# usamec/GAML

Measured on AMD Instinct MI355X. Metric: reads_per_sec_scored, higher is better.
Workload: dtype f64; 1 GPU; cfg3: 5 Mbp, 50x 2x150 paired, insert 300+-30; 833333 pairs in all, whole true genome as 1-2 walks, 8 rotating path sets, window cache warm; pairs_total=833333, pairs_per_gpu=833333, genome_bp=5000000, parallelism=reads sharded over 1 GPU(s)

## Files before the change

gaml_amd/api.py:

```python
from __future__ import annotations

import ctypes as C
import importlib.util
import os
import sys

import numpy as np

_HERE = os.path.dirname(os.path.abspath(__file__))
FLAVOUR = os.environ.get("GAML_HIP_FLAVOUR", "release")
LIB_PATH = os.environ.get("GAML_HIP_LIB") or os.path.join(_HERE, "libgaml_hip_dev.so" if FLAVOUR == "dev" else "libgaml_hip.so")

OK, EINVAL, ENODEVICE, EHIP, ESTATE = 0, -1, -2, -3, -4

_i32p = np.ctypeslib.ndpointer(np.int32, flags="C_CONTIGUOUS")
_i64p = np.ctypeslib.ndpointer(np.int64, flags="C_CONTIGUOUS")
_f64p = np.ctypeslib.ndpointer(np.float64, flags="C_CONTIGUOUS")
_u8p = np.ctypeslib.ndpointer(np.uint8, flags="C_CONTIGUOUS")

ALIGMENT = np.dtype([("position", np.int32), ("edit_dist", np.int32), ("read_id", np.int32), ("orientation", np.int32)])
PACBIO_ALIGMENT = np.dtype([("position", np.int32), ("position_end", np.int32), ("read_id", np.int32), ("pad_", np.int32),
                            ("logprob", np.float64)])


# ... 585 lines not shown
        o = out[:n]
        return np.stack([o["position"], o["edit_dist"], o["read_id"], o["orientation"]], axis=1)

    def align_window(self, rs, mate, walk) -> int:
        walk = np.ascontiguousarray(walk, np.int32)
        return _lib.gaml_hip_align_window(self._h, rs, mate, walk, len(walk))

    def debug_prepare(self, paths):
        flat, offs = _flat(paths)
        self._check(_lib.gaml_hip_debug_prepare(self._h, flat, offs, len(paths)))

    def debug_occurrences(self, rs, mate=0) -> np.ndarray:
        n = _lib.gaml_hip_debug_occurrences(self._h, rs, mate, np.zeros(5, np.int32), 0)
        out = np.zeros(5 * max(1, n), np.int32)
        _lib.gaml_hip_debug_occurrences(self._h, rs, mate, out, n)
        return out.reshape(-1, 5)[:n]

    def debug_table_occurrences(self, rs, mate=0):
        info = np.zeros(3, np.int64)
        n = _lib.gaml_hip_debug_table_occurrences(self._h, rs, mate, np.zeros(5, np.int32), 0, info)
        out = np.zeros(5 * max(1, n), np.int32)
        _lib.gaml_hip_debug_table_occurrences(self._h, rs, mate, out, n, info)
        return out.reshape(-1, 5)[:n], {"incremental": bool(info[0]), "incremental_calls": int(info[1]), "full_calls": int(info[2])}

    def debug_window_walk(self, rs, mate, wid) -> list:
        buf = np.zeros(64, np.int32)
        n = _lib.gaml_hip_debug_window_walk(self._h, rs, mate, wid, buf, 64)
        if n > 64:
            buf = np.zeros(n, np.int32)
            _lib.gaml_hip_debug_window_walk(self._h, rs, mate, wid, buf, n)
        return [int(x) for x in buf[:n]]

    def table_stats(self, rs):
        out = np.zeros(10, np.int64)
        self._check(_lib.gaml_hip_table_stats(self._h, rs, out))
        return {"full_rebuilds": int(out[0]), "delta_updates": int(out[1]), "dirty_pairs": int(out[2]), "worker_rebuilds": int(out[3]), "side_stream_rebuilds": int(out[3]),
                "batches_patched": int(out[4]), "batches_full": int(out[5]), "records_left_out": [int(out[6]), int(out[7])], "delta_records_left_out": int(out[8]),
                "static_index_pairs": int(out[9])}

    def aligner_stats(self):
        w, k, us = C.c_int64(), C.c_int64(), C.c_double()
        _lib.gaml_hip_aligner_stats(self._h, C.byref(w), C.byref(k), C.byref(us))
        return {"windows": w.value, "candidates": k.value, "us": us.value}

    def aligner_stages(self):
        out = np.zeros(6, np.float64)
        self._check(_lib.gaml_hip_aligner_stages(self._h, out))
        return {"strings_upload": out[0], "spans_candidates": out[1], "extension": out[2], "hits_d2h": out[3], "sort_file": out[4], "batches": int(out[5])}

    def last_phases(self):
        out = np.zeros(8, np.float64)
        _lib.gaml_hip_last_phases(self._h, out)
        return out

    def debug_timeline(self, rs: int, cap_waves: int = 1 << 16) -> np.ndarray:
        out = np.zeros((cap_waves, 8), np.uint64)
        n = self._check(_lib.gaml_hip_debug_timeline(self._h, rs, out.ctypes.data, cap_waves))
        return out[:n]

    def debug_set_knob(self, knob, value):
        self._check(_lib.gaml_hip_debug_set_knob(self._h, knob, value))

    def debug_fold_check(self, rs):
        out = np.zeros(6, np.int64)
        self._check(_lib.gaml_hip_debug_fold_check(self._h, rs, out))
        return {"records_left_out": [int(out[0]), int(out[1])], "compact_pairs": [int(out[2]), int(out[3])], "records_checked": int(out[4]),
                "violations": int(out[5])}

    def debug_radix_sort(self, keys, vals=None, begin_bit=0, end_bit=64, running_max=False):
        k = np.ascontiguousarray(keys, np.uint64).copy()
        v = None if vals is None else np.ascontiguousarray(vals, np.uint64).copy()
        m = np.zeros(len(k), np.uint64) if running_max else None
        self._check(_lib.gaml_hip_debug_radix_sort(self._h, k.ctypes.data, None if v is None else v.ctypes.data, len(k), begin_bit, end_bit,
                                                   None if m is None else m.ctypes.data))
        return k, v, m

    def debug_static_check(self, rs):
        out = np.zeros(8, np.int64)
        self._check(_lib.gaml_hip_debug_static_check(self._h, rs, out))
        return {"static_pairs": int(out[0]), "other_pairs": int(out[1]), "violations": int(out[2]), "no_record": int(out[3]),
                "different_windows": int(out[4]), "orientation": int(out[5]), "distance": int(out[6]), "edits_or_code": int(out[7])}

    def debug_occ_route(self, rs):
        out = np.zeros(6, np.int64)
        self._check(_lib.gaml_hip_debug_occ_route(self._h, rs, out))
        return {"device": int(out[0]), "host": int(out[1]), "fallbacks": int(out[2]), "compactions": int(out[3]),
                "pool_entries": int(out[4]), "shared_combinations": int(out[5])}

    def debug_occ_check(self, rs):
        out = np.zeros(4, np.int64)
        rc = _lib.gaml_hip_debug_occ_check(self._h, rs, out)
        res = {"compared": int(out[0]), "present": int(out[1]), "mismatches": int(out[2]), "lists": int(out[3])}
        if rc != 0 and res["compared"] == 0:
            self._check(rc)
        return res

    def debug_tables_check(self, rs):
        out = np.zeros(8, np.int64)
        rc = _lib.gaml_hip_debug_tables_check(self._h, rs, out)
        res = {"pairs": int(out[0]), "compact": int(out[1]), "static": int(out[2]), "two": int(out[3]), "four": int(out[4]), "more": int(out[5]),
               "compared": int(out[6]), "mismatches": int(out[7])}
        if rc != 0 and res["compared"] == 0:
            self._check(rc)
        return res

    def debug_block_partials(self, rs, set_index=0):
        sums, zeros, lay = np.zeros(8192, np.float64), np.zeros(8192, np.int32), np.zeros(8, np.int32)
        _lib.gaml_hip_debug_block_partials.argtypes = [C.c_void_p, C.c_int, C.c_int32, _f64p, _i32p, C.c_int32, _i32p]
        n = _lib.gaml_hip_debug_block_partials(self._h, rs, set_index, sums, zeros, 8192, lay)
        return sums[:max(n, 0)].copy(), zeros[:max(n, 0)].copy(), lay.tolist()

    def pair_classes(self, rs):
        out = np.zeros(4, np.int64)
        self._check(_lib.gaml_hip_pair_classes(self._h, rs, out))
        return out

    debug_table_stats, debug_profile, debug_class_counts = table_stats, last_phases, pair_classes

    def last_timing(self):
        out = np.zeros(3, np.float64)
        _lib.gaml_hip_last_timing(self._h, out)
        return {"host_us": out[0], "device_wall_us": out[1], "kernel_us": out[2]}

    def set_event_timing(self, on):
        _lib.gaml_hip_set_event_timing(self._h, int(on))

    def kernel_stats(self, reset=False):
        n, us, b = C.c_int64(), C.c_double(), C.c_double()
        _lib.gaml_hip_kernel_stats(self._h, 1 if reset else 0, C.byref(n), C.byref(us), C.byref(b))
        return {"launches": n.value, "device_us": us.value, "algo_bytes": b.value}


def debug_sam_band(sam_line: str, total_len: int):
    raw = sam_line.encode()
    f = np.zeros(10, np.int32); r0 = np.zeros(1, np.int32)
    n = _lib.gaml_hip_debug_sam_band(raw, len(raw), total_len, f, r0, np.zeros(1, np.int32), np.zeros(1, np.int32), 0)
    if n < 0:
        raise GamlHipError(n, "malformed SAM line")
    lo = np.zeros(n, np.int32); hi = np.zeros(n, np.int32)
    _lib.gaml_hip_debug_sam_band(raw, len(raw), total_len, f, r0, lo, hi, n)
    keys = ["flags", "len", "posstart", "posend", "sstart", "send", "slen", "tstart", "tend", "edit_dist"]
    return dict(zip(keys, (int(x) for x in f))), int(r0[0]), lo, hi


def debug_sam_shape(sam_line: str, total_len: int):
    raw = sam_line.encode()
    f = np.zeros(6, np.int32)
    n = _lib.gaml_hip_debug_sam_shape(raw, len(raw), total_len, f, None, 0)
    if n < 0:
        raise GamlHipError(n, "malformed SAM line")
    ops = np.zeros(max(1, n), np.uint32)
    _lib.gaml_hip_debug_sam_shape(raw, len(raw), total_len, f, ops.ctypes.data, n)
    keys = ["n_ops", "row_f", "col_f", "bl", "el", "max_width"]
    return dict(zip(keys, (int(x) for x in f))), [(int(o) >> 2, "MID"[int(o) & 3]) for o in ops[:n]]
```

gaml_amd/csrc/ctx.hip.h:

```cpp
#pragma once
#include <hip/hip_runtime.h>
#include <hip/hip_ext.h>
#include "radix_sort.hip.h"

#include <algorithm>
#include <atomic>
#include <fcntl.h>
#include <sys/mman.h>
#include <unistd.h>
#include <chrono>
#include <climits>
#include <limits>
#include <cmath>
#include <cstdio>
#include <cstdlib>
#include <cstring>
#include <immintrin.h>
#include <memory>
#include <set>
#include <string>
#include <thread>
#include <vector>

#include "aligner.hip.h"
// ... 180 lines not shown
    k_in.release(); k_out.release(); k_tmp.release(); v_in.release(); v_tmp.release(); hist.release(); cl.release(); sidx.release(); tiles.release(); peer0.release();
    for (int m = 0; m < 2; m++) { v_sorted[m].release(); rstart[m].release(); rend[m].release(); one[m].release(); more[m].release(); start[m].release(); wins[m].release(); h_wins[m].release(); }
    h_peer.release(); h_cnt.release();
  }
};

struct BuildPlan { int64_t A[2] = {0, 0}; int n_act[2] = {0, 0}; unsigned tiles = 0, none1 = 0, none2 = 0; int ins_n = 0, units = 1; bool empty = true; };

struct TableRebuild {
  bool active = false;
  bool retired = false;
  int next_slice = 0;
  int64_t start_eval = 0;
  TableDev tab;
  hipStream_t stream = nullptr;
  hipEvent_t done = nullptr, mark = nullptr;
  std::vector<std::pair<int32_t, int32_t>> after;
};

struct PairInfo {
  int64_t class_count[4] = {0, 0, 0, 0};
  int64_t n0a = 0;
  std::vector<uint32_t> len_combo;
  int64_t dropped_records[2] = {0, 0};
};

struct PairedSet {
  gaml_paired_cfg cfg;
  ShortMate mate[2];
  PairInfo pt;
  MateDev dev[2];
  TableDev tab;
  TableRebuild rebuild;
  BuildScratch scratch;
  BuildPlan build_plan;
  int64_t async_rebuilds = 0, retired_windows = 0, eval_count = 0;
  DevBuf lcode, len_combo_dev, combo_tabs, memo;
  int memo_codes = 0;
  bool statics_uploaded = false, kernels_warm = false, prereserved = false;
  DevBuf dl_slot, dl_spill, dl_rec[2], sp_rng[2], sp_rec[2], sp_slot, dstate;
  DevBuf dl_bins, dl_bin_count, dl_blk_tot, dl_wlist, dl_stamps;
  PinBuf h_dstate;
  size_t delta_cap = 0, cap_spill = 0, cap_sprec = 0;
  int64_t nd_est = 0, ns_est = 0;
  bool spill_may_grow = false;
  int dl_seq = 0;
  int64_t full_rebuilds = 0, delta_updates = 0;
  int quiet_calls = 0;
  int64_t delta_left_out = 0, delta_left_out_base = 0;
  bool compact_requested = false;
  PinBuf h_timeline; int timeline_waves = 0;
  PinBuf h_part_sum, h_part_zero;
  size_t host_part_stride = 0;
  int last_total_blocks = 0, last_sets = 1;
  int last_blocks[8] = {0, 0, 0, 0, 0, 0, 0, 0};
  bool last_host_partials = false;
  DevBuf probs, tabs, cov_bits, bad;
  Arena arena;
  struct Persist {
    void* dev = nullptr; size_t bytes = 0;
    size_t cap_w[2] = {0, 0}, cap_lo[2] = {0, 0}, cap_m[2] = {0, 0};
    size_t off_tfloor = 0, off_occ[2] = {0, 0}, off_lo[2] = {0, 0}, off_m[2] = {0, 0};
    bool valid = false;
    void release() { if (dev) (void)hipFree(dev); dev = nullptr; bytes = 0; valid = false; }
  } persist;
  struct OccDev {
    DevBuf pool[2];
    size_t pool_cap[2] = {0, 0}, pool_used[2] = {0, 0};
    uint32_t pool_gen = 1;
    PinBuf stage;
    DevBuf tab[2][2], list[2][2];
    DevBuf stamp[2];
    size_t cap_w = 0, cap_list = 0;
    int32_t list_n[2][2] = {{0, 0}, {0, 0}};
    uint32_t serial = 0;
    PinBuf dup;
    bool taken = false;
    bool check_dup = false;
    bool image_stale = false;
    std::vector<std::vector<uint64_t>> shared;
    size_t shared_next = 0;
    std::vector<uint64_t> key;
    int64_t dev_calls = 0, host_calls = 0, fallbacks = 0, compactions = 0;
    void release() {
      for (int mt = 0; mt < 2; mt++) {
        pool[mt].release(); stamp[mt].release();
        for (int k = 0; k < 2; k++) { tab[mt][k].release(); list[mt][k].release(); }
      }
      stage.release(); dup.release();
    }
  } occdev;
  int64_t batches_patched = 0, batches_full = 0;
  size_t batch_slack = 0;
  hipEvent_t ev_tables = nullptr, ev_ovf = nullptr;
  PairedPlanner planner;
  OccImage image[2];
  std::vector<Occ> scratch_occ[2];
  Reducer red;
  Staging stage_pool;
  std::vector<double> ins_tab, floor_tab, logfloor_tab, covthr_tab;
  bool floor_positive = true;
  bool tabs_uploaded = false;
  int64_t last_bad_bases = 0;
};

struct SingleSet {
  gaml_single_cfg cfg;
  ShortMate mate;
  ReadMajor rm;
  MateDev dev;
  DevBuf lens, probs, tabs, occ_arena;
  std::vector<Occ> last_occ;
  Reducer red;
  std::vector<double> floor_tab, logfloor_tab;
  bool tabs_uploaded = false;
  Staging stage;
};

struct DpDev {
  DevBuf path, jobs, ops, scratch, out, dbg;
  void release() { path.release(); jobs.release(); ops.release(); scratch.release(); out.release(); dbg.release(); }
};

struct PbSweepDev {
  DevBuf iv_off, iv;
  std::vector<int32_t> iv_off_host;
  uint64_t generation = ~0ull;
  DevBuf in, all;
  DevBuf key_begin, key_end, pos, key_begin_s, key_end_s, pos_s, end_max, tmp, bad;
  Staging stage;
  void release() {
    iv_off.release(); iv.release(); in.release(); all.release(); key_begin.release(); key_end.release(); pos.release();
    key_begin_s.release(); key_end_s.release(); pos_s.release(); end_max.release(); tmp.release(); bad.release();
    for (int k = 0; k < kRing; k++) { stage.host[k].release(); if (stage.done[k]) (void)hipEventDestroy(stage.done[k]); stage.done[k] = nullptr; stage.armed[k] = false; }
  }
};

struct PacbioSet {
  gaml_single_cfg cfg;
  int64_t n_global = 0, lo = 0, hi = 0;
  std::vector<int32_t> lens;
  double log_match = 0, log_mismatch = 0;
  std::unordered_map<Walk, int32_t, WalkHasher> walk_id;
  std::vector<std::vector<gaml_pacbio_aligment>> recs;
  uint64_t generation = 0, uploaded_generation = ~0ull;
  int32_t max_len = 0;
  int64_t misses = 0;
  DevBuf d_lens, rec_off, rec_walk, rec_logp, walk_count, logprobs;
  Reducer red;
  int64_t last_bad_bases = 0;
  Staging stage;
  PbSweepDev sweep;
  bool have_reads = false;
  std::string bases;
  std::vector<int64_t> base_off;
  std::unordered_map<std::string, int32_t> name_id;
  DevBuf d_bases;
  DpDev dp;
  bool bases_uploaded = false;
  double dp_stats[8] = {0, 0, 0, 0, 0, 0, 0, 0};
};

struct PairedPrep {
  int64_t assembled_records = 0;
  std::vector<int32_t> path_base, start_off, starts;
  int32_t total_bits = 0, n_paths = 0;
  bool general = false;
};

struct SetRef { int kind, idx; };

}
// ... 71 lines not shown
```

gaml_amd/csrc/debug_api.hip.h:

```cpp
#pragma once

int gaml_hip_debug_prepare(gaml_hip_ctx* c, const int32_t* flat, const int64_t* offs, int32_t n_paths) {
  if (!c || n_paths < 0 || (n_paths > 0 && (!flat || !offs))) return fail(c, GAML_HIP_EINVAL, "bad arguments");
  if (c->multi) {
    for (int k = 0; k < gaml::multi_num_shards(c->multi); k++)
      if (int e = gaml_hip_debug_prepare(gaml::multi_shard(c->multi, k), flat, offs, n_paths)) return fail(c, e, gaml_hip_last_error(gaml::multi_shard(c->multi, k)));
    return GAML_HIP_OK;
  }
  if (!c->have_graph) return fail(c, GAML_HIP_ESTATE, "no graph set");
  std::vector<Walk> paths = unflatten(flat, offs, n_paths);
  for (auto& h : scoring_order(c)) {
    if (h.kind == 0) { std::vector<Occ> occs; prepare_single_host(c, *c->singles[h.idx], paths, occs); }
    else if (h.kind == 1) {
      PairedPrep p;
      PairedSet& ps = *c->paireds[h.idx];
      if (int e = prepare_paired_structure(c, ps, flat, offs, n_paths)) return e;
      if (int e = align_pending_pair(c, ps)) return e;
      if (int e = prepare_paired_tables_host(c, ps, p)) return e;
    }
  }
  if (c->peers == 1) {
    for (ShortMate* m : filter_mates(c)) m->unsynced.clear();
  }
  return GAML_HIP_OK;
// ... 202 lines not shown
    paired_base_args(c, s, a, gp);
    layout8[0] = gp.blocks0a; layout8[1] = gp.blocks0; layout8[2] = a.blocks01; layout8[3] = a.blocks012; layout8[4] = a.main_blocks; layout8[5] = a.total_blocks;
    layout8[6] = 0; layout8[7] = n;
  }
  return n;
}



int gaml_hip_debug_tables_check(gaml_hip_ctx* c, int rs, int64_t* out8) {
  MULTI_SHARD0(c);
  if (!c || rs < 0 || rs >= (int)c->handles.size() || c->handles[rs].kind != 1 || !out8) return fail(c, GAML_HIP_EINVAL, "bad arguments");
  if (c->device < 0) return fail(c, GAML_HIP_ENODEVICE, "host-only context");
  PairedSet& s = *c->paireds[c->handles[rs].idx];
  HIP_TRY(c, hipSetDevice(c->device));
  if (s.rebuild.active) { if (int e = paired_build_continue(c, s, true)) return e; HIP_TRY(c, hipEventSynchronize(s.rebuild.done)); s.rebuild.active = false; s.rebuild.after.clear(); }
  if (int e = prepare_paired_tables(c, s)) return e;
  if (int e = pool_mirror(c, s, c->stream)) return e;
  if (int e = paired_upload_statics(c, s, c->stream)) return e;
  TableDev T;
  if (int e = paired_build_enqueue(c, s, T, c->stream)) return e;
  HIP_TRY(c, hipStreamSynchronize(c->stream));
  if (int e = paired_build_collect(c, s, T)) { T.release(); return e; }
  ShortMate hm[2];
  for (int mt = 0; mt < 2; mt++) {
    const ShortMate& m = s.mate[mt];
    hm[mt].n_global = m.n_global; hm[mt].lo = m.lo; hm[mt].hi = m.hi; hm[mt].lens = m.lens;
    hm[mt].wins = m.wins;
    std::vector<int4> dp((size_t)s.dev[mt].pool_n);
    if (!dp.empty()) HIP_TRY(c, hipMemcpy(dp.data(), s.dev[mt].pool.p, dp.size() * sizeof(int4), hipMemcpyDeviceToHost));
    hm[mt].pool.resize(dp.size());
    for (size_t k = 0; k < dp.size(); k++) hm[mt].pool[k] = gaml_aligment{dp[k].y, dp[k].z & 0xff, dp[k].w, (dp[k].z >> 8) & 1};
    for (Window& w : hm[mt].wins) w.first = w.dfirst < 0 ? 0 : w.dfirst;
    for (Window& w : hm[mt].wins) if (w.dfirst < 0) { w.count = 0; }
  }
  PairTables pt;
  build_pair_tables(hm[0], hm[1], pt, KNOB(c, 16) != 1, paired_static_ins_n(c, s));
  const int64_t n = s.mate[0].n_local();
  int64_t compared = 0, bad = 0;
  auto fetch = [&](const DevBuf& d, size_t bytes, std::vector<char>& out) -> int {
    out.resize(bytes);
    if (bytes) HIP_TRY(c, hipMemcpy(out.data(), d.p, bytes, hipMemcpyDeviceToHost));
    return 0;
  };
  auto cmp = [&](const DevBuf& d, const void* host, size_t bytes, size_t elem, const char* what) -> int {
    std::vector<char> v;
    if (int e = fetch(d, bytes, v)) return e;
    int64_t b0 = bad;
    for (size_t k = 0; k < bytes / elem; k++) { compared++; if (memcmp(v.data() + k * elem, (const char*)host + k * elem, elem) != 0) bad++; }
    if (bad != b0 && getenv("GAML_HIP_TRACE_HOST")) fprintf(stderr, "tables_check: %s differs in %lld of %zu entries\n", what, (long long)(bad - b0), bytes / elem);
    return 0;
  };
  for (int k = 0; k < 4; k++) { compared++; bad += T.class_count[k] != pt.class_count[k]; }
  compared++; bad += T.n0a != pt.n0a;
  if (bad == 0) {
    const int64_t n0 = pt.class_count[0], n16 = n - n0;
    if (int e = cmp(T.slot_of_read, pt.slot_of_read.data(), (size_t)n * 4, 4, "slot_of_read")) return e;
    if (int e = cmp(T.read_of_slot, pt.read_of_slot.data(), (size_t)n * 4, 4, "read_of_slot")) return e;
    for (int mt = 0; mt < 2; mt++) {
      if (int e = cmp(T.rec8[mt], pt.rec8[mt].data(), (size_t)n0 * 8, 8, "rec8")) return e;
      if (int e = cmp(T.first[mt], pt.rm[mt].first.data(), (size_t)n16 * 16, 16, "first")) return e;
      if (int e = cmp(T.extra[mt], pt.rm[mt].extra.data(), pt.rm[mt].extra.size() * 16, 16, "extra")) return e;
      if (int e = cmp(T.inl[mt], pt.inl[mt].data(), pt.inl[mt].size() * 16, 16, "inl")) return e;
      compared++; bad += T.extras[mt] != (int64_t)pt.rm[mt].extra.size();
      compared++; bad += T.dropped[mt] != pt.dropped_records[mt];
    }
    if (int e = cmp(T.len_code, pt.len_code.data(), (size_t)n0, 1, "len_code")) return e;
    if (int e = cmp(T.static_idx, pt.static_idx.data(), (size_t)pt.n0a * 4, 4, "static_idx")) return e;
    if (int e = cmp(T.len12, pt.len12.data(), (size_t)n16 * 4, 4, "len12")) return e;
    compared++; bad += pt.len_combo != s.pt.len_combo;
  }
  out8[0] = n; out8[1] = T.class_count[0]; out8[2] = T.n0a; out8[3] = T.class_count[1]; out8[4] = T.class_count[2]; out8[5] = T.class_count[3];
  out8[6] = compared; out8[7] = bad;
  T.release();
  return bad ? fail(c, GAML_HIP_ESTATE, "record tables: the device build differs from the host restatement") : GAML_HIP_OK;
}

int gaml_hip_debug_occ_route(gaml_hip_ctx* c, int rs, int64_t* out6) {
  MULTI_SHARD0(c);
  if (!c || !out6 || rs < 0 || rs >= (int)c->handles.size() || c->handles[rs].kind != 1) return fail(c, GAML_HIP_EINVAL, "bad arguments");
  const PairedSet::OccDev& D = c->paireds[c->handles[rs].idx]->occdev;
  out6[0] = D.dev_calls; out6[1] = D.host_calls; out6[2] = D.fallbacks; out6[3] = D.compactions;
  out6[4] = (int64_t)(D.pool_used[0] + D.pool_used[1]); out6[5] = (int64_t)D.shared.size();
  return GAML_HIP_OK;
}

int gaml_hip_debug_occ_check(gaml_hip_ctx* c, int rs, int64_t* out4) {
  MULTI_SHARD0(c);
  if (!c || !out4 || rs < 0 || rs >= (int)c->handles.size() || c->handles[rs].kind != 1) return fail(c, GAML_HIP_EINVAL, "bad arguments");
  PairedSet& ps = *c->paireds[c->handles[rs].idx];
  const PairedSet::OccDev& D = ps.occdev;
  out4[0] = out4[1] = out4[2] = out4[3] = 0;
  if (!D.image_stale) return GAML_HIP_OK;
  HIP_TRY(c, hipSetDevice(c->device));
  HIP_TRY(c, hipStreamSynchronize(c->stream));
  const PlanView& v = ps.planner.view();
  for (int mt = 0; mt < 2; mt++) {
    OccImage im;
    im.build(ps.mate[mt].wins.size(), v, mt);
    const size_t n = im.occ12.size();
    std::vector<Occ12> dev(n);
    if (n) HIP_TRY(c, hipMemcpy(dev.data(), occdev_table(ps, mt), n * sizeof(Occ12), hipMemcpyDeviceToHost));
    for (size_t w = 0; w < n; w++) {
      const Occ12& h = im.occ12[w];
      const Occ12& d = dev[w];
      const bool absent = h.lo == ~0u && h.hi == ~0u;
      out4[0]++;
      if (!absent) out4[1]++;
      if (absent ? (d.lo != ~0u || d.hi != ~0u) : (d.lo != h.lo || d.hi != h.hi || d.rank != h.rank)) out4[2]++;
    }
    if (!im.general_wids.empty()) out4[3]++;
  }
  if (out4[2] || out4[3]) return fail(c, GAML_HIP_ESTATE, "device occurrence tables differ from the host image");
  return GAML_HIP_OK;
}
```

gaml_amd/csrc/host_model.cc:

```cpp
#include "host_model.h"

#include <algorithm>
#include <chrono>
#include <cmath>
#include <cstdlib>
#include <cstring>
#include <fstream>
#include <thread>

namespace gaml {

void GraphStore::finish() {
  norm.resize(n());
  std::unordered_map<std::string, int32_t> tiny;
  for (int32_t i = 0; i < n(); i++) {
    norm[i] = i;
    if (len(i) > 3) continue;
    std::string s(seq(i), len(i));
    auto it = tiny.find(s);
    if (it == tiny.end()) tiny.emplace(s, i);
    else norm[i] = it->second;
  }
}

// ... 776 lines not shown
    }
    is_new_.assign((size_t)n_paths, 0);
    for (const Edit& e : edits_) for (int32_t k = e.c0; k < e.c1; k++) is_new_[k] = 1;
    for (const Edit& e : edits_) {
      int32_t chain_end = e.c1;
      while (chain_end < n_paths) { const bool has_node = memos_[cur_ids_[chain_end]]->final_last_end != -2; chain_end++; if (has_node) break; }
      registration_chain(g, mate, e.c0, chain_end);
    }
    std::vector<char>& redo = redo_;
    redo.assign(memos_.size(), 0);
    for (int32_t id : in_ids) redo[id] = 1;
    for (int32_t id : stale_) if (id < (int32_t)memos_.size() && memos_[id]->use_count > 0 && (!memos_[id]->valid[0] || !memos_[id]->valid[1] || !memos_[id]->occ_valid[0] || !memos_[id]->occ_valid[1])) redo[id] = 2;
    stale_.clear();
    drain(mate);
    size_t seen = stale_.size();
    for (int32_t k = 0; k < n_paths; k++) {
      const int32_t id = cur_ids_[k];
      if (!redo[id]) continue;
      PathMemo& pm = *memos_[id];
      bool built = false;
      for (int mt = 0; mt < 2; mt++)
        if (!pm.valid[mt]) { build_placements(g, mate[mt], mt, pm, id); built = true; }
      if (!built) continue;
      drain(mate);
      for (; seen < stale_.size(); seen++) {
        const int32_t sid = stale_[seen];
        if (sid >= (int32_t)redo.size() || redo[sid]) continue;
        for (int32_t q = k + 1; q < n_paths; q++) if (cur_ids_[q] == sid) { redo[sid] = 2; break; }
      }
    }
    for (int32_t k = 0; k < n_paths; k++) {
      const int32_t id = cur_ids_[k];
      if (!redo[id]) continue;
      if (!is_new_[k]) {
        const PathMemo& pm = *memos_[id];
        removed_.push_back(Removed{cur_slots_[k], {pm.assembled[0], pm.assembled[1]}, {pm.occ[0], pm.occ[1]}});
      }
      work_.push_back(k);
    }
    std::vector<int32_t> keep;
    for (int32_t sid : stale_) if (sid < (int32_t)memos_.size() && memos_[sid]->use_count > 0 && (!memos_[sid]->valid[0] || !memos_[sid]->valid[1])) keep.push_back(sid);
    stale_.swap(keep);
  }
  const int64_t total = n_paths > 0 ? offs[n_paths] - base : 0;
  prev_flat_.assign(flat + base, flat + base + total);
  prev_offs_.resize((size_t)n_paths + 1);
  for (int32_t k = 0; k <= n_paths; k++) prev_offs_[k] = (n_paths > 0 ? offs[k] : 0) - base;
  have_prev_ = true;
  return true;
}

static void occ_prepack(const std::vector<Occ>& occ, std::vector<OccPre>& pre) {
  pre.resize(occ.size());
  for (size_t k = 0; k < occ.size(); k++) {
    const Occ& o = occ[k];
    const int32_t mp = o.min_pos < -32768 ? -32768 : o.min_pos;
    pre[k] = OccPre{o.min_pos <= 32767 ? o.wid : ~o.wid, (uint32_t)o.shift, (uint32_t)(uint16_t)(int16_t)mp, o.rank};
  }
}

static bool occ_pre_plain(const std::vector<OccPre>& pre) {
  std::vector<int32_t> w(pre.size());
  for (size_t k = 0; k < pre.size(); k++) { if (pre[k].wid < 0) return false; w[k] = pre[k].wid; }
  std::sort(w.begin(), w.end());
  return std::adjacent_find(w.begin(), w.end()) == w.end();
}

void PairedPlanner::invalidate_thresholds() {
  for (auto& pm : memos_) pm->occ_valid[0] = pm->occ_valid[1] = false;
  have_prev_ = false;
}

void PairedPlanner::finish(ShortMate mate[2]) {
  auto redo_occ = [&](PathMemo& pm) {
    for (int mt = 0; mt < 2; mt++) {
      if (pm.occ_valid[mt]) continue;
      pm.occ[mt].clear();
      occurrences_from_placements(mate[mt], pm.pl[mt], pm.occ[mt]);
      pm.assembled[mt] = 0;
      for (const Occ& o : pm.occ[mt]) pm.assembled[mt] += mate[mt].wins[o.wid].count;
      occ_prepack(pm.occ[mt], pm.pre[mt]);
      pm.pre_plain[mt] = occ_pre_plain(pm.pre[mt]);
      pm.dev_off[mt] = -1;
      pm.occ_valid[mt] = true;
    }
  };
  if (!incremental_) {
    for (int32_t id : cur_ids_) redo_occ(*memos_[id]);
    assembled_[0] = assembled_[1] = 0;
    for (int32_t id : cur_ids_) { assembled_[0] += memos_[id]->assembled[0]; assembled_[1] += memos_[id]->assembled[1]; }
  } else {
    for (int32_t k : work_) redo_occ(*memos_[cur_ids_[k]]);
  }
}

const PlanView& PairedPlanner::view() {
  if (!view_valid_) {
    view_.paths.clear();
    for (int32_t id : cur_ids_) view_.paths.push_back(memos_[id].get());
    view_valid_ = true;
  }
  return view_;
}

void PairedPlanner::apply(ShortMate mate[2], OccImage image[2], bool build_image, bool image_stale) {
  if (!incremental_) {
    const PlanView& v = view();
    for (int32_t id : cur_ids_) {
      PathMemo& pm = *memos_[id];
      if (pm.touched_serial == retire_serial_) continue;
      for (int mt = 0; mt < 2; mt++) for (const Occ& o : pm.occ[mt]) mate[mt].touch(o.wid);
      pm.touched_serial = retire_serial_;
    }
    if (build_image) for (int mt = 0; mt < 2; mt++) image[mt].build(mate[mt].wins.size(), v, mt);
    return;
  }
  if (image_stale) {
    for (int mt = 0; mt < 2; mt++) {
      for (const Removed& r : removed_) assembled_[mt] -= r.assembled[mt];
      for (int32_t k : work_) assembled_[mt] += memos_[cur_ids_[k]]->assembled[mt];
    }
    for (int32_t id : cur_ids_) {
      PathMemo& pm = *memos_[id];
      if (pm.touched_serial == retire_serial_) continue;
      for (int mt = 0; mt < 2; mt++) for (const Occ& o : pm.occ[mt]) mate[mt].touch(o.wid);
      pm.touched_serial = retire_serial_;
    }
    rebuild_images(mate, image);
    return;
  }
  for (int32_t k : work_) {
    PathMemo& pm = *memos_[cur_ids_[k]];
    if (pm.touched_serial == retire_serial_) continue;
    for (int mt = 0; mt < 2; mt++) for (const Occ& o : pm.occ[mt]) mate[mt].touch(o.wid);
    pm.touched_serial = retire_serial_;
  }
  if ((int32_t)pos_of_slot_.size() < next_slot_) pos_of_slot_.resize((size_t)next_slot_ + 64, 0);
  for (int32_t k = 0; k < (int32_t)cur_slots_.size(); k++) pos_of_slot_[cur_slots_[k]] = k;
  for (int mt = 0; mt < 2; mt++) {
    OccImage& im = image[mt];
    for (const Removed& r : removed_) { im.remove_path(r.occ[mt], r.slot); assembled_[mt] -= r.assembled[mt]; }
    for (int32_t k : work_) {
      const PathMemo& pm = *memos_[cur_ids_[k]];
      im.add_path(mate[mt].wins.size(), pm.occ[mt], cur_slots_[k]);
      assembled_[mt] += pm.assembled[mt];
    }
    im.finalize(pos_of_slot_);
  }
}

void PairedPlanner::rebuild_images(ShortMate mate[2], OccImage image[2]) {
  if ((int32_t)pos_of_slot_.size() < next_slot_) pos_of_slot_.resize((size_t)next_slot_ + 64, 0);
  for (int32_t k = 0; k < (int32_t)cur_slots_.size(); k++) pos_of_slot_[cur_slots_[k]] = k;
  const PlanView& v = view();
  for (int mt = 0; mt < 2; mt++) image[mt].build(mate[mt].wins.size(), v, mt, &cur_slots_, &pos_of_slot_);
}

void PairedPlanner::mark_used(ShortMate mate[2], const OccImage image[2]) {
  for (int mt = 0; mt < 2; mt++) image[mt].for_each_present([&](int32_t w) { mate[mt].touch(w); });
  for (auto& pm : memos_)
    if (pm->last_used > rebuild_clock_ || pm->use_count > 0)
      for (int mt = 0; mt < 2; mt++) for (const Occ& o : pm->occ[mt]) if (o.wid < (int32_t)mate[mt].wins.size()) mate[mt].touch(o.wid);
}

void PairedPlanner::flat_occurrences(int mate, std::vector<Occ>& out) {
  out.clear();
// ... 646 lines not shown
```

gaml_amd/csrc/host_model.h:

```cpp
#pragma once
#include <climits>
#include <cstdint>
#include <memory>
#include <string>
#include <unordered_map>
#include <vector>

#include "../../include/gaml_hip.h"

namespace gaml {

constexpr int kTail = 300;
constexpr int kSeed = 15;

struct GraphStore {
  std::string bases;
  std::vector<int64_t> off;
  std::vector<int32_t> norm;
  int32_t n() const { return (int32_t)off.size() - 1; }
  int32_t len(int32_t node) const { return (int32_t)(off[node + 1] - off[node]); }
  const char* seq(int32_t node) const { return bases.data() + off[node]; }
  void finish();
  bool load_lastgraph(const std::string& file, std::string* err);
};
// ... 116 lines not shown
#ifndef GAML_FOLD_CLASS2_BELOW
#define GAML_FOLD_CLASS2_BELOW 1024
#endif
constexpr int64_t kFoldClass2Below = GAML_FOLD_CLASS2_BELOW;
constexpr int kMemoCodes = 4;
constexpr int32_t kStaticZero = -2;
constexpr size_t kMemoMaxEntries = (size_t)1 << 24;
#ifdef GAML_HIP_DEV
struct PairTables {
  std::vector<int32_t> slot_of_read, read_of_slot;
  int64_t class_count[4] = {0, 0, 0, 0};
  int64_t n0a = 0;
  std::vector<int32_t> static_idx;
  std::vector<uint64_t> rec8[2];
  std::vector<uint8_t> len_code;
  std::vector<uint32_t> len_combo;
  std::vector<uint32_t> len12;
  ReadMajor rm[2];
  std::vector<RecQuad> inl[2];
  int64_t dropped_records[2] = {0, 0};
};
void build_pair_tables(const ShortMate& a, const ShortMate& b, PairTables& out, bool fold = true, int ins_n = 0);
#endif
void link_mate_windows(ShortMate& a, ShortMate& b);
#ifdef GAML_HIP_DEV
int64_t undominated_records(const ShortMate& m, int32_t wid, std::vector<uint8_t>& keep);
#endif


struct OccQuad { int32_t shift, min_pos, path, rank; };
struct OccTable {
  std::vector<OccQuad> direct;
  std::vector<int32_t> multi_off;
  std::vector<OccQuad> multi;
};
void build_occ_table(size_t n_windows, const std::vector<Occ>& occs, OccTable& out);

void split_contigs(const Walk& path, std::vector<std::pair<int32_t, int32_t>>& ctg_ranges, std::vector<int32_t>& gaps);

struct PlanView;
struct Occ12 { uint32_t lo, hi; int32_t rank; };
struct OccImage {
  std::vector<Occ12> occ12;
  std::vector<int32_t> multi_off;
  std::vector<OccQuad> multi;
  std::vector<int32_t> general_wids;
  void build(size_t n_windows, const PlanView& view, int mate, const std::vector<int32_t>* slots = nullptr,
             const std::vector<int32_t>* pos_of_slot = nullptr);
  void add_path(size_t n_windows, const std::vector<Occ>& occ, int32_t slot);
  void remove_path(const std::vector<Occ>& occ, int32_t slot);
  void finalize(const std::vector<int32_t>& pos_of_slot);
  std::vector<int32_t> changed;
  bool changed_all = true, lists_changed = true;
  void dump(std::vector<Occ>& out) const;
  template <class F> void for_each_present(F f) const { for (int32_t w : touched_) if (cnt_[w] > 0) f(w); }
  void take_changed() { changed.clear(); changed_all = false; lists_changed = false; if (++mark_serial_ == 0) { std::fill(mark_.begin(), mark_.end(), 0); mark_serial_ = 1; } }
 private:
  void grow(size_t n_windows);
  void mark(int32_t w) { if (mark_[w] != mark_serial_) { mark_[w] = mark_serial_; changed.push_back(w); } }
  void set_direct(int32_t w, const OccQuad& q);
  std::vector<int32_t> touched_, stale_, cnt_, list_of_;
  std::vector<uint32_t> stamp_, mark_;
  uint32_t serial_ = 0, mark_serial_ = 1;
  struct Pending { int32_t wid; OccQuad q; };
  std::vector<Pending> pending_;
  std::unordered_map<int32_t, std::vector<OccQuad>> gen_;
  bool lists_dirty_ = false;
};

struct OccPre { int32_t wid; uint32_t lo, hi; int32_t rank; };

struct PathMemo {
  Walk path;
  bool registered[2] = {false, false};
  bool first_pending[2] = {false, false};
  bool valid[2] = {false, false};
  bool occ_valid[2] = {false, false};
  std::vector<Placement> pl[2];
  std::vector<Occ> occ[2];
  std::vector<OccPre> pre[2];
  bool pre_plain[2] = {false, false};
  int64_t dev_off[2] = {-1, -1};
  uint32_t dev_gen[2] = {0, 0};
  int64_t assembled[2] = {0, 0};
  std::vector<int32_t> starts;
  int32_t length = 0;
  int32_t first_idx = -1, first_end = -1;
  int32_t final_last_end = -2;
  int32_t use_count = 0;
  uint32_t touched_serial = 0;
  uint64_t last_used = 0;
  uint32_t serial = 0;
};

struct PlanView {
  std::vector<const PathMemo*> paths;
};

class PairedPlanner {
 public:
  bool begin(const GraphStore& g, ShortMate mate[2], const int32_t* flat, const int64_t* offs, int32_t n_paths,
             bool allow_incremental, std::string* err);
  void finish(ShortMate mate[2]);
  void apply(ShortMate mate[2], OccImage image[2], bool build_image = true, bool image_stale = false);
  void rebuild_images(ShortMate mate[2], OccImage image[2]);
  const std::vector<int32_t>& ids() const { return cur_ids_; }
  PathMemo& memo(int32_t id) { return *memos_[id]; }
  void mark_used(ShortMate mate[2], const OccImage image[2]);
  void note_rebuild(bool retired_some) { rebuild_clock_ = clock_; if (retired_some) retire_serial_++; }
  void invalidate_thresholds();
  void forget_previous() { have_prev_ = false; }
  const PlanView& view();
  void flat_occurrences(int mate, std::vector<Occ>& out);
  size_t memo_count() const { return memos_.size(); }
  int32_t total_len() const { return total_len_; }
  int64_t assembled(int mate) const { return assembled_[mate]; }
  int32_t n_paths() const { return (int32_t)cur_ids_.size(); }
  bool last_was_incremental() const { return incremental_; }
  const std::vector<int32_t>& slots() const { return cur_slots_; }
  uint64_t hits = 0, misses = 0, incremental_calls = 0, full_calls = 0;
 private:
  int32_t lookup_or_create(const GraphStore& g, const int32_t* p, int32_t len, std::string* err);
  void drain(ShortMate mate[2]);
  void build_placements(const GraphStore& g, ShortMate& m, int mt, PathMemo& pm, int32_t id);
  void registration_chain(const GraphStore& g, ShortMate mate[2], int32_t from, int32_t to);
  std::vector<std::unique_ptr<PathMemo>> memos_;
  std::unordered_map<Walk, int32_t, WalkHasher> by_path_;
  std::unordered_map<Walk, std::vector<std::pair<int32_t, uint32_t>>, WalkHasher> missed_[2];
  PlanView view_;
  bool view_valid_ = false;
  std::vector<int32_t> cur_ids_;
  std::vector<int32_t> cur_slots_;
  std::vector<int32_t> free_slots_, pos_of_slot_;
  int32_t next_slot_ = 0;
  std::vector<int32_t> prev_flat_;
  std::vector<int64_t> prev_offs_;
  bool have_prev_ = false;
  bool incremental_ = false;
  struct Removed { int32_t slot; int64_t assembled[2]; std::vector<Occ> occ[2]; };
  std::vector<Removed> removed_;
  std::vector<int32_t> work_;
  std::vector<int32_t> stale_;
  std::vector<char> redo_;
  struct Edit { int32_t p0, p1, c0, c1; };
  std::vector<Edit> edits_;
  std::vector<char> is_new_;
  int32_t total_len_ = 0;
  int64_t assembled_[2] = {0, 0};
  uint64_t clock_ = 0, rebuild_clock_ = 0;
  uint32_t retire_serial_ = 0;
  static constexpr size_t kMaxMemos = 2048;
};
int32_t walk_length(const GraphStore& g, const Walk& w);

bool read_fastq(const std::string& file, std::string& bases, std::vector<int64_t>& offs, std::string* err,
                std::vector<std::string>* names = nullptr);

struct SamRecord {
  std::string name;
  int32_t flags = 0, len = 0, posstart = 0, posend = 0, sstart = 0, send = 0, slen = 0, tstart = 0, tend = 0, edit_dist = 0;
  std::vector<std::pair<int32_t, char>> cigar;
};
bool parse_sam_record(const char* begin, const char* end, int32_t total_len, SamRecord& out);

struct DpBand {
  int32_t row0 = 0, max_width = 0;
// ... 11 lines not shown
```

gaml_amd/csrc/kernels.hip.h:

```cpp
#pragma once
#include <hip/hip_runtime.h>
#include <stdint.h>

namespace gaml {

constexpr int kBlock = 256;
constexpr int kMaxBlocks = 2048;
enum { kDsDirty = 0, kDsSpill = 1, kDsTop0 = 2, kDsTop1 = 3, kDsOverflow = 4, kDsSeq = 5, kDsInts = 8 };

__device__ __forceinline__ unsigned long long occ8_of(const Occ12* t, unsigned w) { const Occ12* e = t + w; return (unsigned long long)e->lo | ((unsigned long long)e->hi << 32); }

struct MateView {
  const int4* first;
  const int4* extra;
  const int4* occ;
  const Occ12* occ12;
  const int* multi_off;
  const int4* multi;
  const double* mism_pow;
  const double* match_pow;
};

struct PairedArgs {
  int total_blocks, blocks0a, n0a, n_codes;
  int blocks0;
  int blocks01, blocks012;
  int main_blocks;
  const double2* memo;
  uint32_t* cov_bits;
  const unsigned long long* rec8[2];
  const double2* static_val;
  const Occ12* occ12[2];
  double* probs;
  double* part_sum;
  int* part_zero;
  double log_two_T;
  double tfloor0, logfloor0;
  uint32_t len_combo0; int pad0_;
  MateView m[2];
  const uint32_t* len12;
  const double* ins_tab;
  int ins_n;
  const double* floor_tab;
  const double* logfloor_tab;
  const double* covthr_tab;
  double two_T;
  int n;
  const int* path_base;
  const unsigned char* len_code;
  const uint32_t* len_combo;
  const double* pe[2];
  const double* floor_c;
  const double* logfloor_c;
  const double* covthr_c;
  int lt_codes;
  const double* tfloor_c;
  const int4* inl[2];
  int n0;
  const int* static_idx;
  int n01;
  int n_main;
  unsigned long long* timeline;
  const int* dstate;
  const int* dirty_slots;
  const int4* dirty_recs[2];
  const int* dirty_spill;
  const int2* spill_rng[2];
  const int4* spill_recs[2];
  const int* spill_slot;
  unsigned* ticket;
  double* out;
  double n_reads;
  double* status_out;
  double status_a, status_b;
};

struct Cand { int path, pos, edit, orient, rank, k; bool valid; };

__device__ __forceinline__ int4 occ_from_compact(unsigned long long o, int rk) {
  const int4 e = make_int4((int)(unsigned)o, (int)(short)(o >> 32), (int)((o >> 48) & 0x7fff), rk);
  return o == ~0ull ? make_int4(0, 0, -1, 0) : e;
}
__device__ __forceinline__ int4 mate_occ(const MateView& v, int w) {
  if (v.occ) return v.occ[w];
  const Occ12 e = v.occ12[w];
  return occ_from_compact((unsigned long long)e.lo | ((unsigned long long)e.hi << 32), e.rank);
}

__device__ __forceinline__ Cand make_cand(const int4& r, const int4& o, int k) {
  Cand c;
  c.path = o.z; c.pos = r.y + o.x; c.edit = r.z & 0xff; c.orient = (r.z >> 8) & 1;
  c.rank = o.w; c.k = k; c.valid = r.y >= o.y;
  return c;
}

struct TableSrc {
  const MateView* v;
  int4 r0;
  __device__ __forceinline__ int count() const { return r0.x < 0 ? 0 : 1 + (int)((unsigned)r0.z >> 9); }
  __device__ __forceinline__ int4 get(int k) const { return k == 0 ? r0 : v->extra[r0.w + k - 1]; }
};
struct ListSrc {
  const int4* recs;
  int cnt;
  __device__ __forceinline__ int count() const { return cnt; }
  __device__ __forceinline__ int4 get(int k) const { return recs[k]; }
};

template <class Src, class F>
__device__ __forceinline__ void for_each_cand_src(const MateView& v, const Src& src, F f) {
  const int cnt = src.count();
  for (int k = 0; k < cnt; k++) {
    int4 r = src.get(k);
    if (r.x < 0) continue;
    int4 o = mate_occ(v, r.x);
    if (o.z < 0) continue;
    if (o.w >= 0) {
      f(make_cand(r, o, k));
    } else {
      const int s = -o.w - 1;
      for (int q = v.multi_off[s]; q < v.multi_off[s + 1]; q++) f(make_cand(r, v.multi[q], k));
    }
  }
}
template <class F>
__device__ __forceinline__ void for_each_cand(const MateView& v, const int4& r0, F f) {
  for_each_cand_src(v, TableSrc{&v, r0}, f);
}

template <class Src>
__device__ __forceinline__ bool is_live_src(const MateView& v, const Src& src, const Cand& c) {
  if (!c.valid) return false;
  bool live = true;
  for_each_cand_src(v, src, [&](const Cand& d) {
    if (d.valid && d.path == c.path && d.pos == c.pos && (d.rank > c.rank || (d.rank == c.rank && d.k > c.k))) live = false;
  });
  return live;
}
__device__ __forceinline__ bool is_live(const MateView& v, const int4& r0, const Cand& c) {
  return is_live_src(v, TableSrc{&v, r0}, c);
}

__device__ __forceinline__ void mark_bit(uint32_t* bits, int bit) {
  atomicOr(&bits[bit >> 5], 1u << (bit & 31));
}

__device__ __forceinline__ double pair_term(const PairedArgs& a, const Cand& x, const Cand& y, int L1, int L2) {
  if (x.orient == y.orient) return 0.0;
  int dist;
  if (x.pos < y.pos) {
    if (x.orient != 0 || y.orient != 1) return 0.0;
    dist = y.pos - x.pos + L2;
  } else {
    if (x.orient != 1 || y.orient != 0) return 0.0;
    dist = x.pos - y.pos + L1;
  }
  if ((unsigned)dist >= (unsigned)a.ins_n) return 0.0;
  double p1 = a.m[0].mism_pow[x.edit] * a.m[0].match_pow[L1 - x.edit];
  double p2 = a.m[1].mism_pow[y.edit] * a.m[1].match_pow[L2 - y.edit];
  double ip = a.ins_tab[dist];
  double t = p1 * p2 * ip;
  if (a.cov_bits && t > a.covthr_tab[L2]) {
    int base = a.path_base[x.path];
    mark_bit(a.cov_bits, base + max(x.pos, y.pos));
    mark_bit(a.cov_bits, base + min(x.pos, y.pos));
  }
  return t;
}
// ... 37 lines not shown
      const bool ly = (live2 >> iy) & 1ull;
      iy++;
      if (!ly || y.path != x.path) return;
      acc += pair_term(a, x, y, L1, L2);
    });
  });
  return acc;
}
template <class Src>
__device__ __forceinline__ double paired_general_src(const PairedArgs& a, const Src& s1, const Src& s2, int L1, int L2) {
  return paired_general_src_slow(a, s1, s2, L1, L2);
}
__device__ __forceinline__ double paired_general(const PairedArgs& a, const int4& r1, const int4& r2, int L1, int L2) {
  return paired_general_src_masks(a, TableSrc{&a.m[0], r1}, TableSrc{&a.m[1], r2}, L1, L2);
}

__device__ __forceinline__ void block_reduce(double& s, int& z, double* sh_s, int* sh_z) {
  for (int off = 32; off > 0; off >>= 1) {
    s += __shfl_down(s, off, 64);
    z += __shfl_down(z, off, 64);
  }
  const int lane = threadIdx.x & 63, wave = threadIdx.x >> 6;
  if (lane == 0) { sh_s[wave] = s; sh_z[wave] = z; }
  __syncthreads();
  if (threadIdx.x == 0) {
    double ts = 0; int tz = 0;
    for (int w = 0; w < kBlock / 64; w++) { ts += sh_s[w]; tz += sh_z[w]; }
    s = ts; z = tz;
  }
}

constexpr int kTicketWords = 17;
__device__ __forceinline__ void grid_finish(double s, int z, int my_slot, int n_partials, double* part_sum, int* part_zero,
                                            unsigned* ticket, double* out, double bad_bases, double n_reads, double* sh_s, int* sh_z,
                                            double* status_out = nullptr, double status_a = 0.0, double status_b = 0.0) {
  __shared__ bool is_last;
  if (threadIdx.x == 0) {
    __hip_atomic_store(&part_sum[my_slot], s, __ATOMIC_RELAXED, __HIP_MEMORY_SCOPE_AGENT);
    __hip_atomic_store(&part_zero[my_slot], z, __ATOMIC_RELAXED, __HIP_MEMORY_SCOPE_AGENT);
    asm volatile("s_waitcnt vmcnt(0)" ::: "memory");
    const int g = my_slot & 15;
    const unsigned in_group = (unsigned)((n_partials - g + 15) >> 4), groups = (unsigned)min(16, n_partials);
    bool last = false;
    if (__hip_atomic_fetch_add(&ticket[1 + g], 1u, __ATOMIC_RELAXED, __HIP_MEMORY_SCOPE_AGENT) == in_group - 1)
      last = __hip_atomic_fetch_add(&ticket[0], 1u, __ATOMIC_RELAXED, __HIP_MEMORY_SCOPE_AGENT) == groups - 1;
    is_last = last;
  }
  __syncthreads();
  if (!is_last) return;
  double ts = 0; int tz = 0;
  for (int b = threadIdx.x; b < n_partials; b += kBlock) {
    ts += __hip_atomic_load(&part_sum[b], __ATOMIC_RELAXED, __HIP_MEMORY_SCOPE_AGENT);
    tz += __hip_atomic_load(&part_zero[b], __ATOMIC_RELAXED, __HIP_MEMORY_SCOPE_AGENT);
  }
  __syncthreads();
  block_reduce(ts, tz, sh_s, sh_z);
  if (threadIdx.x < kTicketWords) __hip_atomic_store(&ticket[threadIdx.x], 0u, __ATOMIC_RELAXED, __HIP_MEMORY_SCOPE_AGENT);
  if (threadIdx.x == 0) {
    out[0] = ts;
    out[1] = (double)tz;
    if (bad_bases >= 0) out[2] = bad_bases;
    out[3] = n_reads;
    if (status_out) { status_out[0] = status_a; status_out[1] = status_b; }
  }
}

struct PairVal { double t, logt; int key, kind; };

__device__ __forceinline__ void finish_read(const PairedArgs& a, int i, double acc, int L1, int L2, double& lsum, int& zeros, PairVal* cap = nullptr) {
  if (cap) *cap = PairVal{acc, 0.0, L1 + L2, 3};
  a.probs[i] = acc;
  const double p = acc / a.two_T;
  const int s = L1 + L2;
  if (p < a.floor_tab[s]) { zeros++; lsum += a.logfloor_tab[s]; }
  else lsum += log(p);
}

template <int K>
struct RegCands {
  int path[K], pos[K], ef[K], rank[K];
  bool valid[K], live[K];
};

template <int K>
__device__ __forceinline__ bool cands_from_records(const MateView& v, const int4 (&r)[K], RegCands<K>& c) {
  int4 o[K];
  bool multi = false;
  Occ12 e[K];
#pragma unroll
  for (int k = 0; k < K; k++) e[k] = v.occ12[r[k].x >= 0 ? r[k].x : 0];
#pragma unroll
  for (int k = 0; k < K; k++) o[k] = occ_from_compact((unsigned long long)e[k].lo | ((unsigned long long)e[k].hi << 32), e[k].rank);
#pragma unroll
  for (int k = 0; k < K; k++) if (r[k].x < 0) o[k] = make_int4(0, 0, -1, 0);
#pragma unroll
  for (int k = 0; k < K; k++) {
    multi |= (o[k].z >= 0 && o[k].w < 0);
    c.path[k] = o[k].z; c.pos[k] = r[k].y + o[k].x; c.ef[k] = r[k].z & 0x1ff; c.rank[k] = o[k].w;
    c.valid[k] = r[k].x >= 0 && o[k].z >= 0 && r[k].y >= o[k].y;
  }
#pragma unroll
  for (int i = 0; i < K; i++) {
    bool lv = c.valid[i];
#pragma unroll
    for (int j = 0; j < K; j++)
      if (j != i) lv = lv && !(c.valid[j] && c.path[j] == c.path[i] && c.pos[j] == c.pos[i] &&
                               (c.rank[j] > c.rank[i] || (c.rank[j] == c.rank[i] && j > i)));
    c.live[i] = lv;
  }
  return multi;
}
template <int K>
__device__ __forceinline__ bool load_cands_inline(const MateView& v, const int4* rec, RegCands<K>& c) {
  int4 r[K];
#pragma unroll
  for (int k = 0; k < K; k++) r[k] = rec[k];
  return cands_from_records<K>(v, r, c);
}

template <int K>
__device__ __forceinline__ double score_regs(const PairedArgs& a, const RegCands<K>& c1, const RegCands<K>& c2, int L1, int L2) {
  int n1 = 0, n2 = 0;
  Cand x, y;
  x.path = -1; x.pos = 0; x.edit = 0; x.orient = 0; y = x;
#pragma unroll
  for (int i = 0; i < K; i++) {
    if (c1.live[i]) { n1++; x.path = c1.path[i]; x.pos = c1.pos[i]; x.edit = c1.ef[i] & 0xff; x.orient = c1.ef[i] >> 8; }
    if (c2.live[i]) { n2++; y.path = c2.path[i]; y.pos = c2.pos[i]; y.edit = c2.ef[i] & 0xff; y.orient = c2.ef[i] >> 8; }
  }
  if (n1 == 0 || n2 == 0) return 0.0;
  if (n1 == 1 && n2 == 1) return x.path == y.path ? pair_term(a, x, y, L1, L2) : 0.0;
  double acc = 0.0;
#pragma unroll
  for (int i = 0; i < K; i++) {
#pragma unroll
    for (int j = 0; j < K; j++) {
      if (c1.live[i] && c2.live[j] && c1.path[i] == c2.path[j]) {
        Cand x, y;
        x.path = c1.path[i]; x.pos = c1.pos[i]; x.edit = c1.ef[i] & 0xff; x.orient = c1.ef[i] >> 8;
        y.path = c2.path[j]; y.pos = c2.pos[j]; y.edit = c2.ef[j] & 0xff; y.orient = c2.ef[j] >> 8;
        acc += pair_term(a, x, y, L1, L2);
      }
    }
  }
  return acc;
}

constexpr unsigned long long kNone8 = ~0ull;
constexpr unsigned long long kDirty8 = ~0ull - 1;
constexpr int kDirtyWid = -2;

__device__ __forceinline__ int4 rec8_to_quad(unsigned long long r) {
  if (r == kNone8 || r == kDirty8) return make_int4(r == kDirty8 ? kDirtyWid : -1, 0, 0, 0);
  return make_int4((int)(r & 0xffffff), (int)((r >> 24) & 0xfffffff), (int)((r >> 52) & 63) | ((int)((r >> 58) & 1) << 8), 0);
}

struct Compact1 {
  unsigned long long r1, r2, o1, o2;
  int L1, L2, lc;
};

__global__ __launch_bounds__(kBlock) void logterm_kernel(const double* pe0, const double* pe1, const double* ins_tab, int ins_n, int codes,
                                                        double2* memo) {
  const int total = codes * 49 * ins_n;
  for (int idx = blockIdx.x * kBlock + threadIdx.x; idx < total; idx += gridDim.x * kBlock) {
    const int dist = idx % ins_n;
    const int q = idx / ins_n;
    const int e2 = q % 7, e1 = (q / 7) % 7, code = q / 49;
    const double t = pe0[code * 64 + e1] * pe1[code * 64 + e2] * ins_tab[dist];
    memo[idx] = make_double2(t, log(t));
  }
}

// ... 82 lines not shown
      for (int q = 0; q < K; q++) {
        const Cand y = make_cand(r2, e2[q], 0);
        if (q >= l2.n || !y.valid || y.path != x.path) continue;
        acc += pair_term(a, x, y, L1, L2);
      }
    }
  } else {
    for (int p = 0; p < l1.n; p++) {
      const Cand x = make_cand(r1, l1.e[p], 0);
      if (!x.valid) continue;
      for (int q = 0; q < l2.n; q++) {
        const Cand y = make_cand(r2, l2.e[q], 0);
        if (!y.valid || y.path != x.path) continue;
        acc += pair_term(a, x, y, L1, L2);
      }
    }
  }
  finish_read_compact(a, i, acc, lc, lsum, zeros);
}

struct GenOut { double add; int zeros; };
__device__ GenOut compact_general_call(unsigned long long kernargs, int i, int set);
__device__ GenOut general_pair_call(unsigned long long kernargs, int i, int dj, int set, int4* lds);
__device__ __forceinline__ unsigned long long kernel_args_address() {
#if defined(__HIP_DEVICE_COMPILE__)
  return (unsigned long long)__builtin_amdgcn_kernarg_segment_ptr();
#else
  return 0;
#endif
}

__device__ __forceinline__ void compact_finish(const PairedArgs& a, int i, const Compact1& c, const CompactPrep& q, double2 m,
                                               double& lsum, int& zeros, PairVal* cap = nullptr) {
  if (q.memo_idx >= 0) {
    const double t = m.x;
    if (cap) *cap = PairVal{t, m.y, c.lc, 1};
    compact_cover(a, c, q, t);
    __builtin_nontemporal_store(t, &a.probs[i]);
    const bool floored = t < a.tfloor_c[c.lc];
    lsum += floored ? a.logfloor_c[c.lc] : m.y - a.log_two_T;
    zeros += (int)floored;
    return;
  }
  double t = 0.0;
  if (q.scores) { t = compact_term_tables(a, c, q); compact_cover(a, c, q, t); }
  finish_read_compact(a, i, t, c.lc, lsum, zeros, cap);
}

__device__ __forceinline__ void finish_val(const PairedArgs& a, int i, const PairVal& v, bool store, double& lsum, int& zeros) {
  if (v.kind == 0) return;
  if (store) __builtin_nontemporal_store(v.t, &a.probs[i]);
  if (v.kind == 1) {
    const bool floored = v.t < a.tfloor_c[v.key];
    lsum += floored ? a.logfloor_c[v.key] : v.logt - a.log_two_T;
    zeros += (int)floored;
  } else if (v.kind == 2) {
    if (v.t == 0.0 && a.floor_c[v.key] > 0.0) { zeros++; lsum += a.logfloor_c[v.key]; return; }
    const double p = v.t / a.two_T;
    if (p < a.floor_c[v.key]) { zeros++; lsum += a.logfloor_c[v.key]; }
    else lsum += log(p);
  } else {
    const double p = v.t / a.two_T;
    if (p < a.floor_tab[v.key]) { zeros++; lsum += a.logfloor_tab[v.key]; }
    else lsum += log(p);
  }
}

__device__ __forceinline__ void compact_load(const PairedArgs& a, int i, bool ok, Compact1& c) {
  c.r1 = ok ? a.rec8[0][i] : kNone8;
  c.r2 = ok ? a.rec8[1][i] : kNone8;
  c.lc = ok ? a.len_code[i] : 0;
}

#if defined(GAML_HIP_DEV) && defined(GAML_GEN_X)
#define GAML_GEN_OFF(bit) ((GAML_GEN_X) & (bit))
#else
#define GAML_GEN_OFF(bit) 0
#endif
struct SlotRange { int lo, hi, lb, blocks; };
__device__ __forceinline__ SlotRange compact_range(const PairedArgs& a, int lb) {
  return lb < a.blocks0a ? SlotRange{0, a.n0a, lb, a.blocks0a} : SlotRange{a.n0a, a.n0, lb - a.blocks0a, a.blocks0 - a.blocks0a};
}

template <bool GEN>
__device__ __forceinline__ void paired_compact_body(const PairedArgs& a, const SlotRange rg, double& lsum, int& zeros) {
  const int stride = rg.blocks * kBlock, hi = rg.hi;
  int i0 = rg.lo + rg.lb * kBlock + threadIdx.x;
  if (i0 >= hi) return;
  Compact1 c0, c1;
  compact_load(a, i0, true, c0);
  compact_load(a, i0 + stride, i0 + stride < hi, c1);
  while (true) {
    const int i1 = i0 + stride;
    const bool two = i1 < hi;
    const int j0 = i0 + 2 * stride;
    const bool more = j0 < hi;
    Compact1 n0v, n1v;
    compact_load(a, j0, more, n0v);
    compact_load(a, j0 + stride, j0 + stride < hi, n1v);
    const uint32_t l0 = a.len_combo[c0.lc], l1 = a.len_combo[c1.lc];
    c0.L1 = l0 & 0xffff; c0.L2 = l0 >> 16; c1.L1 = l1 & 0xffff; c1.L2 = l1 >> 16;
    const bool d0 = c0.r1 == kDirty8, d1 = c1.r1 == kDirty8;
    if (d0) { c0.r1 = kNone8; c0.r2 = kNone8; }
    if (d1) { c1.r1 = kNone8; c1.r2 = kNone8; }
    c0.o1 = c0.r1 != kNone8 ? occ8_of(a.occ12[0], (unsigned)(c0.r1 & 0xffffff)) : kNone8;
    c0.o2 = c0.r2 != kNone8 ? occ8_of(a.occ12[1], (unsigned)(c0.r2 & 0xffffff)) : kNone8;
    c1.o1 = c1.r1 != kNone8 ? occ8_of(a.occ12[0], (unsigned)(c1.r1 & 0xffffff)) : kNone8;
    c1.o2 = c1.r2 != kNone8 ? occ8_of(a.occ12[1], (unsigned)(c1.r2 & 0xffffff)) : kNone8;
    CompactPrep q0, q1;
    compact_prep(a, c0, q0);
    compact_prep(a, c1, q1);
    const double2 m0 = q0.memo_idx >= 0 ? a.memo[q0.memo_idx] : make_double2(0.0, 0.0);
    const double2 m1 = q1.memo_idx >= 0 ? a.memo[q1.memo_idx] : make_double2(0.0, 0.0);
    if (!d0 && !q0.skip) compact_finish(a, i0, c0, q0, m0, lsum, zeros);
    else if (GEN && q0.skip) { const GenOut o = compact_general_call(kernel_args_address(), i0, -1); lsum += o.add; zeros += o.zeros; }
    if (two && !d1 && !q1.skip) compact_finish(a, i1, c1, q1, m1, lsum, zeros);
    else if (GEN && two && q1.skip) { const GenOut o = compact_general_call(kernel_args_address(), i1, -1); lsum += o.add; zeros += o.zeros; }
    if (!more) break;
    c0 = n0v; c1 = n1v;
    i0 = j0;
  }
}

constexpr int kPairZero = -1, kPairOther = -(1 << 20);
__device__ __forceinline__ int compact_state(const PairedArgs& a, uint2 r1, uint2 r2, uint2 o1, uint2 o2, unsigned lc, uint32_t l12,
                                             bool in_range, bool& skip) {
  const bool v1 = r1.y != ~0u, v2 = r2.y != ~0u;
  const bool w1 = v1 & (o1.y != ~0u), w2 = v2 & (o2.y != ~0u);
  const bool here = in_range & !(r1.y == ~0u && r1.x == 0xfffffffeu);
  skip = here & ((w1 & ((int)o1.y < 0)) | (w2 & ((int)o2.y < 0)));
  const int L1 = l12 & 0xffff, L2 = l12 >> 16;
  const int p1 = (int)(__funnelshift_r(r1.x, r1.y, 24) & 0xfffffffu), p2 = (int)(__funnelshift_r(r2.x, r2.y, 24) & 0xfffffffu);
  const int x = p1 + (int)o1.x, y = p2 + (int)o2.x;
  const unsigned or1 = (r1.y >> 26) & 1u, or2 = (r2.y >> 26) & 1u;
  const bool fwd = x < y;
  const int dist = fwd ? y - x + L2 : x - y + L1;
  const bool scores = w1 & w2 & !skip & (((o1.y ^ o2.y) >> 16) == 0)
                      & (p1 >= (int)(short)(o1.y & 0xffffu)) & (p2 >= (int)(short)(o2.y & 0xffffu))
                      & (or1 != or2) & (or1 == (fwd ? 0u : 1u));
  const unsigned e1 = (r1.y >> 20) & 63u, e2 = (r2.y >> 20) & 63u;
  const bool in_memo = scores & ((unsigned)dist < (unsigned)a.ins_n) & (lc < (unsigned)a.lt_codes) & (e1 < 7u) & (e2 < 7u);
  const int idx = (int)((lc * 7u + e1) * 7u + e2) * a.ins_n + dist;
  int state = in_memo ? idx : ((skip | scores) ? kPairOther : kPairZero - (int)lc);
  if (!here) state = kPairOther - 1;
  return state;
}

template <bool GEN, bool TL = false, bool ONE = false>
__device__ __forceinline__ void paired_compact4_body(const PairedArgs& a, const SlotRange rg, double& lsum, int& zeros) {
  const unsigned stride = (unsigned)rg.blocks * kBlock, n0 = (unsigned)rg.hi;
  unsigned long long* tl = TL ? a.timeline + ((size_t)blockIdx.x * (kBlock / 64) + (threadIdx.x >> 6)) * 8 : nullptr;
#define GAML_STAMP(slot, dep) if (TL) { asm volatile("s_waitcnt vmcnt(0)" ::: "memory"); if ((threadIdx.x & 63) == 0) tl[slot] = (unsigned long long)wall_clock64() + ((dep) == 0x12345u ? 1 : 0); }
  const char* const rec0 = (const char*)a.rec8[0];
  const char* const rec1 = (const char*)a.rec8[1];
  const char* const occ0 = (const char*)a.occ12[0];
  const char* const occ1 = (const char*)a.occ12[1];
  const char* const memo = (const char*)a.memo;
  char* const probs = (char*)a.probs;
  const uint32_t l12_one = ONE ? a.len_combo[0] : 0u;
  const double logfloor_one = ONE ? a.logfloor_c[0] : 0.0, tfloor_one = ONE ? a.tfloor_c[0] : 0.0, log2T = a.log_two_T;
  for (unsigned base = (unsigned)rg.lo + (unsigned)rg.lb * kBlock + threadIdx.x; base < n0; base += 4 * stride) {
    uint2 r1[4], r2[4], o1[4], o2[4];
    unsigned lc[4];
#pragma unroll
    for (int k = 0; k < 4; k++) {
      const unsigned ic = base + k * stride < n0 ? base + k * stride : base;
      r1[k] = *(const uint2*)(rec0 + ic * 8u); r2[k] = *(const uint2*)(rec1 + ic * 8u); lc[k] = ONE ? 0u : (unsigned)a.len_code[ic];
    }
    GAML_STAMP(2, r1[0].x ^ r1[1].x ^ r1[2].x ^ r1[3].x ^ r2[0].x ^ r2[3].x)
#pragma unroll
    for (int k = 0; k < 4; k++) {
      const Occ12* e1 = (const Occ12*)(occ0 + (r1[k].y != ~0u ? (r1[k].x & 0xffffffu) : 0u) * 12u);
      const Occ12* e2 = (const Occ12*)(occ1 + (r2[k].y != ~0u ? (r2[k].x & 0xffffffu) : 0u) * 12u);
      o1[k] = make_uint2(e1->lo, e1->hi); o2[k] = make_uint2(e2->lo, e2->hi);
    }
    GAML_STAMP(3, o1[0].x ^ o1[1].x ^ o1[2].x ^ o1[3].x ^ o2[0].x ^ o2[3].x)
    int state[4];
    unsigned skip_bits = 0;
#pragma unroll
    for (int k = 0; k < 4; k++) {
      bool skip;
      state[k] = compact_state(a, r1[k], r2[k], o1[k], o2[k], lc[k], ONE ? l12_one : a.len_combo[lc[k]], base + k * stride < n0, skip);
      skip_bits |= (unsigned)skip << k;
    }
    double2 m[4];
#pragma unroll
    for (int k = 0; k < 4; k++) m[k] = *(const double2*)(memo + (unsigned)max(state[k], 0) * 16u);
    GAML_STAMP(4, (unsigned)(__double2loint(m[0].x) ^ __double2loint(m[1].x) ^ __double2loint(m[2].x) ^ __double2loint(m[3].x)))
    bool other = false;
#pragma unroll
    for (int k = 0; k < 4; k++) {
      double* const out = (double*)(probs + (base + k * stride) * 8u);
      if (state[k] >= 0) {
        __builtin_nontemporal_store(m[k].x, out);
        const bool floored = m[k].x < (ONE ? tfloor_one : a.tfloor_c[lc[k]]);
        lsum += floored ? (ONE ? logfloor_one : a.logfloor_c[lc[k]]) : m[k].y - log2T;
        zeros += (int)floored;
      } else if (state[k] > kPairOther) {
        __builtin_nontemporal_store(0.0, out);
        zeros++;
        lsum += ONE ? logfloor_one : a.logfloor_c[kPairZero - state[k]];
      } else other |= state[k] == kPairOther && !((skip_bits >> k) & 1u);
    }
    GAML_STAMP(5, 0u)
    if (__any(other)) {
#pragma unroll 1
      for (int k = 0; k < 4; k++) {
        if (state[k] != kPairOther || ((skip_bits >> k) & 1u)) continue;
        const int i = (int)(base + k * stride);
        Compact1 d;
        compact_load(a, i, true, d);
        d.o1 = d.r1 != kNone8 ? occ8_of(a.occ12[0], (unsigned)(d.r1 & 0xffffff)) : kNone8;
        d.o2 = d.r2 != kNone8 ? occ8_of(a.occ12[1], (unsigned)(d.r2 & 0xffffff)) : kNone8;
        const uint32_t l = a.len_combo[d.lc];
        d.L1 = l & 0xffff; d.L2 = l >> 16;
        CompactPrep q;
        compact_prep(a, d, q);
        compact_finish(a, i, d, q, make_double2(0.0, 0.0), lsum, zeros);
      }
    }
    if (GEN && !GAML_GEN_OFF(8) && __any(skip_bits != 0)) {
#pragma unroll 1
      for (int k = 0; k < 4; k++)
        if ((skip_bits >> k) & 1u) { const GenOut o = compact_general_call(kernel_args_address(), (int)(base + k * stride), -1); lsum += o.add; zeros += o.zeros; }
    }
  }
#undef GAML_STAMP
}

#ifndef GAML_LEAN_ENTRY
#define GAML_LEAN_ENTRY 1
#endif
#if GAML_LEAN_ENTRY && defined(__HIP_DEVICE_COMPILE__)
#define GAML_FRESH_ARGS(name, fallback)                                                                                   \
  const __attribute__((address_space(4))) PairedArgs* name##_p =                                                          \
      (const __attribute__((address_space(4))) PairedArgs*)__builtin_amdgcn_kernarg_segment_ptr();                        \
  asm volatile("" : "+s"(name##_p));                                                                                      \
  const PairedArgs name = *name##_p;
#else
#define GAML_FRESH_ARGS(name, fallback) const PairedArgs& name = fallback;
#endif
#ifndef GAML_STATIC_P
#define GAML_STATIC_P 4
#endif
#ifndef GAML_STATIC_PIPE
#define GAML_STATIC_PIPE 0
#endif
#if defined(GAML_HIP_DEV) && defined(GAML_STATIC_X)
#define GAML_TIMING_X(bit) ((GAML_STATIC_X) & (bit))
#else
#define GAML_TIMING_X(bit) 0
#endif
__global__ __launch_bounds__(kBlock) void static_values_kernel(const int* static_idx, int n0a, const double2* memo, double2* static_val) {
  for (int i = blockIdx.x * kBlock + threadIdx.x; i < n0a; i += gridDim.x * kBlock) {
    const int mi = static_idx[i];
    static_val[i] = mi >= 0 ? memo[mi] : make_double2(0.0, 0.0);
  }
}

template <bool GEN, bool TL = false, bool ONE = false>
__device__ __forceinline__ void paired_static4_body(const PairedArgs& a, const SlotRange rg, double& lsum, int& zeros) {
  constexpr int P = GAML_STATIC_P;
  const unsigned stride = (unsigned)rg.blocks * kBlock, n0 = (unsigned)rg.hi;
  unsigned long long* tl = TL ? a.timeline + ((size_t)blockIdx.x * (kBlock / 64) + (threadIdx.x >> 6)) * 8 : nullptr;
#define GAML_STAMP(slot, dep) if (TL && first_round) { asm volatile("s_waitcnt vmcnt(0)" ::: "memory"); if ((threadIdx.x & 63) == 0) tl[slot] = (unsigned long long)wall_clock64() + ((dep) == 0x12345u ? 1 : 0); }
  const char* const rec0 = (const char*)a.rec8[0];
  const char* const rec1 = (const char*)a.rec8[1];
  const char* const sval = (const char*)a.static_val;
  const char* const occ0 = (const char*)a.occ12[0];
  const char* const occ1 = (const char*)a.occ12[1];
  char* const probs = (char*)a.probs;
  const double logfloor_one = ONE ? a.logfloor0 : 0.0, tfloor_one = ONE ? a.tfloor0 : 0.0, log2T = a.log_two_T;
  unsigned base = (unsigned)rg.lo + (unsigned)rg.lb * kBlock + threadIdx.x;
  if (base >= n0) return;
  uint2 r1[P], r2[P];
  double2 m[P];
  unsigned lc[P];
#pragma unroll
  for (int k = 0; k < P; k++) {
    const unsigned ic = base + k * stride < n0 ? base + k * stride : base;
    r1[k] = *(const uint2*)(rec0 + ic * 8u); r2[k] = *(const uint2*)(rec1 + ic * 8u); m[k] = GAML_TIMING_X(4) ? make_double2(1e-9 * (double)ic, -20.0) : *(const double2*)(sval + ic * 16u);
    lc[k] = ONE ? 0u : (unsigned)a.len_code[ic];
  }
  bool first_round = true;
  while (true) {
    GAML_STAMP(2, r1[0].x ^ r2[0].x ^ (unsigned)__double2loint(m[0].x))
    uint2 o1[P], o2[P];
#pragma unroll
    for (int k = 0; k < P; k++) {
      const unsigned w1 = (r1[k].x & 0xffffffu) & (0u - (unsigned)(r1[k].y != ~0u)), w2 = (r2[k].x & 0xffffffu) & (0u - (unsigned)(r2[k].y != ~0u));
      const Occ12* e1 = (const Occ12*)(occ0 + w1 * 12u);
      const Occ12* e2 = (const Occ12*)(occ1 + w2 * 12u);
      o1[k] = make_uint2(e1->lo, e1->hi); o2[k] = make_uint2(e2->lo, e2->hi);
      if (GAML_TIMING_X(1)) { o1[k] = make_uint2(r1[k].x >> 8, 0u); o2[k] = make_uint2(r1[k].x >> 8, 0u); }
    }
    const unsigned nbase = base + P * stride;
    const bool more = nbase < n0;
    uint2 nr1[P], nr2[P];
    double2 nm[P];
    unsigned nlc[P];
    if (GAML_STATIC_PIPE && __any(more)) {
#pragma unroll
      for (int k = 0; k < P; k++) {
        const unsigned ic = nbase + k * stride < n0 ? nbase + k * stride : base;
        nr1[k] = *(const uint2*)(rec0 + ic * 8u); nr2[k] = *(const uint2*)(rec1 + ic * 8u); nm[k] = *(const double2*)(sval + ic * 16u);
        nlc[k] = ONE ? 0u : (unsigned)a.len_code[ic];
      }
    }
    GAML_STAMP(3, o1[0].x ^ o2[0].x)
    GAML_STAMP(4, 0u)
    unsigned skip_bits = 0;
#pragma unroll
    for (int k = 0; k < P; k++) {
      const bool none1 = r1[k].y == ~0u, none2 = r2[k].y == ~0u;
      const bool here = (base + k * stride < n0) & !(none1 & (r1[k].x == 0xfffffffeu));
      const bool w1 = !none1 & (o1[k].y != ~0u), w2 = !none2 & (o2[k].y != ~0u);
      const bool gen = here & ((w1 & ((int)o1[k].y < 0)) | (w2 & ((int)o2[k].y < 0)));
      const bool same = (o1[k].x == o2[k].x) & (((o1[k].y ^ o2[k].y) >> 16) == 0);
      const int p1 = (int)(__funnelshift_r(r1[k].x, r1[k].y, 24) & 0xfffffffu), p2 = (int)(__funnelshift_r(r2[k].x, r2[k].y, 24) & 0xfffffffu);
      const bool kept = (p1 >= (int)(short)(o1[k].y & 0xffffu)) & (p2 >= (int)(short)(o2[k].y & 0xffffu));
      const bool both = here & !gen & w1 & w2;
      const bool scores = both & same & kept;
      const bool poison = both & !same;
      const bool counted = here & !gen;
      skip_bits |= (unsigned)gen << k;
      const double t = scores ? m[k].x : 0.0;
      const bool floored = counted & (!scores | (t < (ONE ? tfloor_one : a.tfloor_c[lc[k]])));
      const double lf = ONE ? logfloor_one : a.logfloor_c[lc[k]];
      double add = floored ? lf : m[k].y - log2T;
      add = counted ? add : 0.0;
      add = poison ? __builtin_nan("") : add;
      lsum += add;
      zeros += (int)floored;
      if (counted && !GAML_TIMING_X(2)) __builtin_nontemporal_store(t, (double*)(probs + (base + k * stride) * 8u));
    }
    if (GEN && !GAML_GEN_OFF(1) && __any(skip_bits != 0)) {
#pragma unroll 1
      for (int k = 0; k < P; k++)
        if ((skip_bits >> k) & 1u) { const GenOut o = compact_general_call(kernel_args_address(), (int)(base + k * stride), -1); lsum += o.add; zeros += o.zeros; }
    }
    GAML_STAMP(5, 0u)
    first_round = false;
    if (!more) break;
    base = nbase;
    if (GAML_STATIC_PIPE) {
#pragma unroll
      for (int k = 0; k < P; k++) { r1[k] = nr1[k]; r2[k] = nr2[k]; m[k] = nm[k]; lc[k] = nlc[k]; }
    } else {
#pragma unroll
      for (int k = 0; k < P; k++) {
        const unsigned ic = base + k * stride < n0 ? base + k * stride : base;
        r1[k] = *(const uint2*)(rec0 + ic * 8u); r2[k] = *(const uint2*)(rec1 + ic * 8u); m[k] = GAML_TIMING_X(4) ? make_double2(1e-9 * (double)ic, -20.0) : *(const double2*)(sval + ic * 16u);
        lc[k] = ONE ? 0u : (unsigned)a.len_code[ic];
      }
    }
  }
#undef GAML_STAMP
}

#ifndef GAML_GEN_CANDS
#define GAML_GEN_CANDS 32
#endif
constexpr int kGenCands = GAML_GEN_CANDS;
#ifdef GAML_GEN_STAMPS
__device__ unsigned long long g_gen_stamp[32];
#define GEN_STAMP(k) do { asm volatile("s_waitcnt vmcnt(0) lgkmcnt(0)" ::: "memory"); const unsigned long long now_ = wall_clock64(); \
  if (__ffsll((long long)__ballot(1)) - 1 == (int)(threadIdx.x & 63)) atomicAdd(&g_gen_stamp[k], now_ - gen_t_); atomicMax(&g_gen_stamp[16 + k], now_ - gen_t_); if (now_ - gen_t_ > 1000) atomicAdd(&g_gen_stamp[24 + k], 1ull); gen_t_ = now_; } while (0)
#define GEN_STAMP_BEGIN unsigned long long gen_t_ = wall_clock64(); const unsigned long long gen_t0_ = gen_t_; if (__ffsll((long long)__ballot(1)) - 1 == (int)(threadIdx.x & 63)) atomicAdd(&g_gen_stamp[15], 1ull);
#else
#define GEN_STAMP(k) do { } while (0)
#define GEN_STAMP_BEGIN
#endif
constexpr int kGenListBatch = 8;
template <int K>
__device__ __forceinline__ bool general_pair_staged(const PairedArgs& a, const int4 (&r1)[K], const int4 (&r2)[K], int L1, int L2, double& acc_out, int4* cand) {
  int n[2] = {0, 0};
// ... 53 lines not shown
          if (q < left) cm[n[m] + q] = make_int4(t[q].z, pos[q], (r.z & 0x1ff) | (((valid >> q) & 1u) ? 0x200 : 0) | (k << 10), t[q].w);
        if (left > 0) { live[m] |= nl << n[m]; n[m] += min(left, kGenListBatch); }
      }
    }
  }
  GEN_STAMP(2);
#ifdef GAML_GEN_STAMPS
  if (!fits) atomicAdd(&g_gen_stamp[12], 1ull);
#endif
  if (!fits) return false;
  GEN_STAMP(3);
  double acc = 0.0;
  for (int x = 0; x < n[0]; x++) {
    if (!((live[0] >> x) & 1u)) continue;
    const int4 cx = cand[x];
    Cand X; X.path = cx.x; X.pos = cx.y; X.edit = cx.z & 0xff; X.orient = (cx.z >> 8) & 1;
    for (int y = 0; y < n[1]; y++) {
      if (!((live[1] >> y) & 1u)) continue;
      const int4 cy = cand[kGenCands + y];
      if (cy.x != cx.x) continue;
      Cand Y; Y.path = cy.x; Y.pos = cy.y; Y.edit = cy.z & 0xff; Y.orient = (cy.z >> 8) & 1;
      acc += pair_term(a, X, Y, L1, L2);
    }
  }
  GEN_STAMP(4);
#ifdef GAML_GEN_STAMPS
  if (__ffsll((long long)__ballot(1)) - 1 == (int)(threadIdx.x & 63)) { atomicAdd(&g_gen_stamp[8], (unsigned long long)n[0]); atomicAdd(&g_gen_stamp[9], (unsigned long long)n[1]); atomicAdd(&g_gen_stamp[10], (unsigned long long)__popc(live[0])); atomicAdd(&g_gen_stamp[11], (unsigned long long)__popcll(__ballot(1))); }
  atomicMax(&g_gen_stamp[13], wall_clock64() - gen_t0_); atomicMax(&g_gen_stamp[14], (unsigned long long)(n[0] * 1000 + n[1])); atomicMax(&g_gen_stamp[7], (unsigned long long)(__popc(live[0]) * 1000 + __popc(live[1])));
#endif
  acc_out = acc;
  return true;
}
constexpr int kOvfCap = 128;
constexpr int kGenWaveSlots = 2 * kOvfCap / (2 * kGenCands);
__device__ __forceinline__ int4* gen_wave_slot(int4* wave_lds, bool mine) {
  const unsigned long long m = __ballot(mine);
  const int rank = __popcll(m & ((1ull << (threadIdx.x & 63)) - 1ull));
  return (wave_lds && mine && rank < kGenWaveSlots) ? wave_lds + rank * 2 * kGenCands : nullptr;
}

template <int K>
__device__ __forceinline__ void score_cands_and_finish(const PairedArgs& a, int i, uint32_t l12, const RegCands<K>& x, const RegCands<K>& y,
                                                       double& lsum, int& zeros, PairVal* cap = nullptr) {
  const int L1 = l12 & 0xffff, L2 = l12 >> 16;
    if (a.memo) {
      int n1 = 0, n2 = 0;
      Compact1 c;
      CompactPrep q;
      q.x.path = -1; q.x.pos = 0; q.x.edit = 0; q.x.orient = 0; q.y = q.x;
#pragma unroll
      for (int k = 0; k < K; k++) {
        if (x.live[k]) { n1++; q.x.path = x.path[k]; q.x.pos = x.pos[k]; q.x.edit = x.ef[k] & 0xff; q.x.orient = x.ef[k] >> 8; }
        if (y.live[k]) { n2++; q.y.path = y.path[k]; q.y.pos = y.pos[k]; q.y.edit = y.ef[k] & 0xff; q.y.orient = y.ef[k] >> 8; }
      }
      int code = (a.lt_codes > 0 && l12 == a.len_combo0) ? 0 : -1;
      if (code < 0 && a.n_codes > 1) {
#pragma unroll
        for (int k = 3; k >= 1; k--) if (k < a.lt_codes && a.len_combo[k] == l12) code = k;
      }
      if (n1 == 1 && n2 == 1 && q.x.path == q.y.path && code >= 0 && q.x.orient != q.y.orient && q.x.edit < 7 && q.y.edit < 7) {
        const bool fwd = q.x.pos < q.y.pos;
        const bool ok = fwd ? (q.x.orient == 0) : (q.x.orient == 1);
        const int dist = fwd ? q.y.pos - q.x.pos + L2 : q.x.pos - q.y.pos + L1;
        if (ok && dist >= 0 && dist < a.ins_n) {
          c.lc = code; c.L1 = L1; c.L2 = L2;
          q.dist = dist; q.scores = true; q.skip = false;
          q.memo_idx = ((code * 7 + q.x.edit) * 7 + q.y.edit) * a.ins_n + dist;
          const double tfl = code == 0 ? a.tfloor0 : a.tfloor_c[code], lfl = code == 0 ? a.logfloor0 : a.logfloor_c[code];
          const double2 m = a.memo[q.memo_idx];
          if (cap) *cap = PairVal{m.x, m.y, code, 1};
          compact_cover(a, c, q, m.x);
          __builtin_nontemporal_store(m.x, &a.probs[i]);
          const bool floored = m.x < tfl;
          lsum += floored ? lfl : m.y - a.log_two_T;
          zeros += (int)floored;
          return;
        }
      }
    }
    const double acc = score_regs<K>(a, x, y, L1, L2);
    finish_read(a, i, acc, L1, L2, lsum, zeros, cap);
}

template <int K, bool GEN>
__device__ __forceinline__ void paired_regs_body(const PairedArgs& a, int lb, int slot_lo, int slot_hi, int block_lo, int block_hi,
                                                 double& lsum, int& zeros, unsigned long long* tl = nullptr, int4* wave_lds = nullptr) {
  bool first_pair = true;
#ifdef GAML_GEN_STAMPS
  const unsigned long long tb_ = wall_clock64();
#endif
  for (int i = slot_lo + (lb - block_lo) * kBlock + threadIdx.x; i < slot_hi; i += (block_hi - block_lo) * kBlock) {
    const int t = i - a.n0;
    const uint32_t l12 = a.len12[t];
    const size_t at = K == 2 ? (size_t)2 * (i - a.n0) : (size_t)2 * (a.n01 - a.n0) + (size_t)4 * (i - a.n01);
    int4 r1[K], r2[K];
#pragma unroll
    for (int k = 0; k < K; k++) { r1[k] = a.inl[0][at + k]; r2[k] = a.inl[1][at + k]; }
    if (tl && first_pair) { asm volatile("s_waitcnt vmcnt(0)" ::: "memory"); if ((threadIdx.x & 63) == 0) tl[2] = (unsigned long long)wall_clock64() + (r1[0].x == 0x12345 ? 1 : 0); }
    RegCands<K> x, y;
    const bool m1 = cands_from_records<K>(a.m[0], r1, x), m2 = cands_from_records<K>(a.m[1], r2, y);
    if (tl && first_pair) { asm volatile("s_waitcnt vmcnt(0)" ::: "memory"); if ((threadIdx.x & 63) == 0) tl[3] = (unsigned long long)wall_clock64() + (x.pos[0] == 0x12345 ? 1 : 0); }
    const bool dirty = r1[0].x == kDirtyWid;
    const bool general = !dirty && (m1 || m2);
    if (!dirty && !general) score_cands_and_finish<K>(a, i, l12, x, y, lsum, zeros);
    if (tl && first_pair) { asm volatile("s_waitcnt vmcnt(0)" ::: "memory"); if ((threadIdx.x & 63) == 0) tl[5] = (unsigned long long)wall_clock64() + (lsum == 0.12345 ? 1 : 0); }
    first_pair = false;
    if (GEN && !GAML_GEN_OFF(2) && __any(general)) {
      int4* const slot = gen_wave_slot(wave_lds, general);
#ifdef GAML_GEN_STAMPS
      const unsigned long long tc0_ = wall_clock64();
#endif
      if (general) {
        double acc;
        const int L1 = l12 & 0xffff, L2 = l12 >> 16;
        int4 priv[K == 2 ? 2 * kGenCands : 1];
        if (K == 2 && general_pair_staged<K>(a, r1, r2, L1, L2, acc, slot ? slot : priv)) finish_read(a, i, acc, L1, L2, lsum, zeros);
        else { const GenOut o = general_pair_call(kernel_args_address(), i, -1, -1, slot); lsum += o.add; zeros += o.zeros; }
      }
#ifdef GAML_GEN_STAMPS
      if (general) { asm volatile("s_waitcnt vmcnt(0) lgkmcnt(0)" ::: "memory"); const unsigned long long tc1_ = wall_clock64(); atomicAdd(&g_gen_stamp[5], tc1_ - tc0_); atomicAdd(&g_gen_stamp[6], 1ull); atomicAdd(&g_gen_stamp[21], tc0_ - tb_); }
#endif
    }
  }
}

template <bool GEN>
__device__ __forceinline__ void paired_delta_body(const PairedArgs& a, int db, int delta_blocks, double& lsum, int& zeros, int4* wave_lds = nullptr) {
  for (int dj = db * kBlock + threadIdx.x; dj < a.dstate[kDsDirty]; dj += delta_blocks * kBlock) {
    const int i = a.dirty_slots[dj];
    const int sp = a.dirty_spill[dj];
    int4 r0[4], r1[4];
#pragma unroll
    for (int k = 0; k < 2; k++) { r0[k] = a.dirty_recs[0][4 * (size_t)dj + k]; r1[k] = a.dirty_recs[1][4 * (size_t)dj + k]; }
    const uint32_t l12 = (uint32_t)r0[0].w;
    const int c0 = r1[0].w & 0xff, c1 = (r1[0].w >> 8) & 0xff;
    bool general = false;
    if (__all(sp >= 0 || (c0 <= 2 && c1 <= 2))) {
      if (sp < 0) {
        RegCands<2> x, y;
        const int4 q0[2] = {r0[0], r0[1]}, q1[2] = {r1[0], r1[1]};
        const bool m0 = cands_from_records<2>(a.m[0], q0, x), m1 = cands_from_records<2>(a.m[1], q1, y);
        general = m0 || m1;
        if (!general) score_cands_and_finish<2>(a, i, l12, x, y, lsum, zeros);
      }
    } else if (sp < 0) {
#pragma unroll
      for (int k = 2; k < 4; k++) { r0[k] = a.dirty_recs[0][4 * (size_t)dj + k]; r1[k] = a.dirty_recs[1][4 * (size_t)dj + k]; }
      RegCands<4> x, y;
      const bool m0 = cands_from_records<4>(a.m[0], r0, x), m1 = cands_from_records<4>(a.m[1], r1, y);
      general = m0 || m1;
      if (!general) score_cands_and_finish<4>(a, i, l12, x, y, lsum, zeros);
    }
    if (GEN) {
      if (!GAML_GEN_OFF(4) && __any(general)) {
        int4* const slot = gen_wave_slot(wave_lds, general);
        if (general) { const GenOut o = general_pair_call(kernel_args_address(), i, dj, -1, slot); lsum += o.add; zeros += o.zeros; }
      }
    } else if (general) {
      lsum += __builtin_nan("");
    }
  }
}

struct DeltaPatch { int dj, slot, spill, pad; int4 rec[2][4]; };
struct DeltaPatch2 { int dj, slot, spill, pad; int4 rec[2][2]; };
__device__ __forceinline__ void mark_dirty_slot(int s, unsigned long long* rec8_0, int n0, int4* inl_0, int n01, int n_main, int4* first_0) {
  if (s < n0) rec8_0[s] = ~0ull - 1;
  else {
    if (s < n01) inl_0[(size_t)2 * (s - n0)].x = -2;
    else if (s < n_main) inl_0[(size_t)2 * (n01 - n0) + (size_t)4 * (s - n01)].x = -2;
    first_0[s - n0].x = -2;
  }
}
template <class Patch, int K>
__global__ __launch_bounds__(kBlock) void apply_delta_patch_kernel(const Patch* patch, int n, int* slots, int* spill, int4* rec0, int4* rec1, int mark_from,
                                                                   unsigned long long* rec8_0, int n0, int4* inl_0, int n01, int n_main, int4* first_0) {
  for (int t = blockIdx.x * kBlock + threadIdx.x; t < n; t += gridDim.x * kBlock) {
    const Patch p = patch[t];
    slots[p.dj] = p.slot;
    spill[p.dj] = p.spill;
#pragma unroll
    for (int k = 0; k < 4; k++) {
      rec0[4 * (size_t)p.dj + k] = k < K ? p.rec[0][k < K ? k : 0] : make_int4(-1, 0, 0, 0);
      rec1[4 * (size_t)p.dj + k] = k < K ? p.rec[1][k < K ? k : 0] : make_int4(-1, 0, 0, 0);
    }
    if (mark_from >= 0 && p.dj >= mark_from) mark_dirty_slot(p.slot, rec8_0, n0, inl_0, n01, n_main, first_0);
  }
}

template <bool TICKET, bool GEN, bool TL>
__device__ __forceinline__ void paired_main_body(const PairedArgs& a, int lb, double* sh_s, int* sh_z, int4* gen_lds) {
  double lsum = 0.0;
  int zeros = 0;
  unsigned long long* tl = TL ? a.timeline + ((size_t)blockIdx.x * (kBlock / 64) + (threadIdx.x >> 6)) * 8 : nullptr;
  if (TL && (threadIdx.x & 63) == 0) { tl[0] = wall_clock64(); tl[7] = lb < a.blocks0 ? 0 : (lb < a.blocks01 ? 1 : 2); }
  if (GAML_TIMING_X(8) && lb >= a.blocks0a) {
  } else if (GAML_TIMING_X(16) && lb < a.blocks0a) {
  } else if (lb < a.blocks0) {
    GAML_FRESH_ARGS(c, a)
    const bool wide = c.memo && !c.cov_bits;
    const SlotRange rg = compact_range(c, lb);
    const bool stat = wide && lb < c.blocks0a;
    if (!TL && wide && c.n_codes == 1) {
      if (stat) paired_static4_body<GEN, false, true>(c, rg, lsum, zeros);
      else paired_compact4_body<GEN, false, true>(c, rg, lsum, zeros);
    } else {
      __shared__ uint32_t sh_combo[256];
      __shared__ double sh_floor[256], sh_logfloor[256], sh_tfloor[256];
      for (int k = threadIdx.x; k < c.n_codes; k += kBlock) { sh_combo[k] = c.len_combo[k]; sh_floor[k] = c.floor_c[k]; sh_logfloor[k] = c.logfloor_c[k]; sh_tfloor[k] = c.tfloor_c ? c.tfloor_c[k] : 0.0; }
      __syncthreads();
      PairedArgs b = c;
      b.len_combo = sh_combo; b.floor_c = sh_floor; b.logfloor_c = sh_logfloor; b.tfloor_c = sh_tfloor;
      if (TL && (threadIdx.x & 63) == 0) tl[1] = wall_clock64();
      if (stat) paired_static4_body<GEN, TL>(b, rg, lsum, zeros);
      else if (wide) paired_compact4_body<GEN, TL>(b, rg, lsum, zeros);
      else paired_compact_body<GEN>(b, rg, lsum, zeros);
    }
  } else {
    int4* const wave_lds = GEN ? gen_lds + (threadIdx.x >> 6) * 2 * kOvfCap : nullptr;
    if (lb < a.blocks01) {
      GAML_FRESH_ARGS(c, a)
      paired_regs_body<2, GEN>(c, lb, c.n0, c.n01, c.blocks0, c.blocks01, lsum, zeros, tl, wave_lds);
    } else if (lb < a.blocks012) {
      GAML_FRESH_ARGS(c, a)
      paired_regs_body<4, GEN>(c, lb, c.n01, c.n_main, c.blocks01, c.blocks012, lsum, zeros, nullptr, wave_lds);
    } else {
      GAML_FRESH_ARGS(c, a)
      paired_delta_body<GEN>(c, lb - c.blocks012, c.main_blocks - c.blocks012, lsum, zeros, wave_lds);
    }
  }
  block_reduce(lsum, zeros, sh_s, sh_z);
  if (TL && (threadIdx.x & 63) == 0) tl[6] = wall_clock64();
  if (TICKET) {
    GAML_FRESH_ARGS(c, a)
    grid_finish(lsum, zeros, lb, c.total_blocks, c.part_sum, c.part_zero, c.ticket, c.out,
                c.cov_bits ? -1.0 : 0.0, c.n_reads, sh_s, sh_z, c.status_out, c.status_a, c.status_b);
  } else if (threadIdx.x == 0) {
    a.part_sum[lb] = lsum;
    a.part_zero[lb] = zeros;
  }
}

__global__ __launch_bounds__(kBlock) void finish_partials_kernel(const double* part_sum, const int* part_zero, int n_partials,
                                                                 double* out, double bad_bases, double n_reads,
                                                                 double* status_out = nullptr, double status_a = 0.0, double status_b = 0.0) {
  __shared__ double sh_s[kBlock / 64];
  __shared__ int sh_z[kBlock / 64];
  double ts = 0; int tz = 0;
  for (int b = threadIdx.x; b < n_partials; b += kBlock) { ts += part_sum[b]; tz += part_zero[b]; }
  block_reduce(ts, tz, sh_s, sh_z);
  if (threadIdx.x == 0) {
    out[0] = ts; out[1] = (double)tz; if (bad_bases >= 0) out[2] = bad_bases; out[3] = n_reads;
    if (status_out) { status_out[0] = status_a; status_out[1] = status_b; }
  }
}

constexpr int kOvfMaxBlocks = 1024;

template <class Src>
__device__ __forceinline__ int wave_gather(const MateView& v, const Src& src, int4* lds, int lane) {
  const int cnt = src.count();
  int total = 0;
  for (int base = 0; base < cnt; base += 64) {
    const int k = base + lane;
    int mine = 0;
    int4 r = make_int4(-1, 0, 0, 0), o = make_int4(0, 0, -1, 0);
    if (k < cnt) {
      r = src.get(k);
      if (r.x >= 0) { const Occ12 e = v.occ12[r.x]; o = occ_from_compact((unsigned long long)e.lo | ((unsigned long long)e.hi << 32), e.rank); }
      if (o.z >= 0) mine = o.w >= 0 ? 1 : v.multi_off[-o.w] - v.multi_off[-o.w - 1];
    }
    int incl = mine;
    for (int d = 1; d < 64; d <<= 1) { int t = __shfl_up(incl, d, 64); if (lane >= d) incl += t; }
    const int wave_total = __shfl(incl, 63, 64);
    const int at = total + incl - mine;
    if (total + wave_total > kOvfCap) return -1;
    if (mine == 1 && o.w >= 0) {
      lds[at] = make_int4(o.z, r.y + o.x, (r.z & 0x1ff) | ((r.y >= o.y) ? 0x200 : 0), o.w);
    } else if (mine > 0) {
      const int s = -o.w - 1;
      for (int q = 0; q < mine; q++) {
        const int4 oo = v.multi[v.multi_off[s] + q];
        lds[at + q] = make_int4(oo.z, r.y + oo.x, (r.z & 0x1ff) | ((r.y >= oo.y) ? 0x200 : 0), oo.w);
      }
    }
    total += wave_total;
  }
  return total;
}

template <class Src>
__device__ __forceinline__ double wave_score_pair(const PairedArgs& a, const Src& s1, const Src& s2, int L1, int L2, int4* c1, int4* c2, int lane) {
  const int n1 = wave_gather(a.m[0], s1, c1, lane);
  const int n2 = wave_gather(a.m[1], s2, c2, lane);
  double acc = 0.0;
  if (n1 < 0 || n2 < 0) {
    if (lane == 0) acc = paired_general_src(a, s1, s2, L1, L2);
    return acc;
  }
  __builtin_amdgcn_wave_barrier();
  for (int m = 0; m < 2; m++) {
    int4* c = m == 0 ? c1 : c2;
    const int n = m == 0 ? n1 : n2;
    for (int x = lane; x < n; x += 64) {
      int4 me = c[x];
      bool live = (me.z & 0x200) != 0;
      for (int y = 0; y < n && live; y++) {
        const int4 ot = c[y];
        if (y != x && (ot.z & 0x200) && ot.x == me.x && ot.y == me.y && (ot.w > me.w || (ot.w == me.w && y > x))) live = false;
      }
      if (live) me.z |= 0x400;
      c[x].z = me.z;
    }
  }
  __builtin_amdgcn_wave_barrier();
  const int pairs = n1 * n2;
  for (int idx = lane; idx < pairs; idx += 64) {
    const int4 xr = c1[idx / n2];
    const int4 yr = c2[idx % n2];
    if ((xr.z & 0x400) && (yr.z & 0x400) && xr.x == yr.x) {
      Cand x, y;
      x.path = xr.x; x.pos = xr.y; x.edit = xr.z & 0xff; x.orient = (xr.z >> 8) & 1;
      y.path = yr.x; y.pos = yr.y; y.edit = yr.z & 0xff; y.orient = (yr.z >> 8) & 1;
      acc += pair_term(a, x, y, L1, L2);
    }
  }
  for (int off = 32; off > 0; off >>= 1) acc += __shfl_xor(acc, off, 64);
  __builtin_amdgcn_wave_barrier();
  return acc;
}

template <bool TICKET>
__device__ __forceinline__ void paired_overflow_body(const PairedArgs& a, int ovf_block, int ovf_blocks, double* sh_s, int* sh_z,
                                                     int4 (*cand)[2][kOvfCap]) {
  const int lane = threadIdx.x & 63, wave = threadIdx.x >> 6;
  const int wave_global = ovf_block * (kBlock / 64) + wave;
  const int n_waves = ovf_blocks * (kBlock / 64);
  const int n_table = a.n - a.n_main;
  const int n_items = n_table + a.dstate[kDsSpill];
  double lsum = 0.0;
  int zeros = 0;
  int4* c1 = cand[wave][0];
  int4* c2 = cand[wave][1];
  for (int item = wave_global; item < n_items; item += n_waves) {
    if (item < n_table) {
      const int i = a.n_main + item;
      const int4 r1 = a.m[0].first[i - a.n0], r2 = a.m[1].first[i - a.n0];
      const uint32_t l12 = a.len12[i - a.n0];
      if (r1.x == kDirtyWid) continue;
      const int L1 = l12 & 0xffff, L2 = l12 >> 16;
      const double acc = wave_score_pair(a, TableSrc{&a.m[0], r1}, TableSrc{&a.m[1], r2}, L1, L2, c1, c2, lane);
      if (lane == 0) finish_read(a, i, acc, L1, L2, lsum, zeros);
    } else {
      const int sp = item - n_table;
      const int i = a.spill_slot[sp];
      const uint32_t l12 = i < a.n0 ? a.len_combo[a.len_code[i]] : a.len12[i - a.n0];
      const int L1 = l12 & 0xffff, L2 = l12 >> 16;
      const int2 g0 = a.spill_rng[0][sp], g1 = a.spill_rng[1][sp];
      const double acc = wave_score_pair(a, ListSrc{a.spill_recs[0] + g0.x, g0.y}, ListSrc{a.spill_recs[1] + g1.x, g1.y}, L1, L2, c1, c2, lane);
      if (lane == 0) finish_read(a, i, acc, L1, L2, lsum, zeros);
    }
  }
  block_reduce(lsum, zeros, sh_s, sh_z);
  if (TICKET) {
    grid_finish(lsum, zeros, a.main_blocks + ovf_block, a.total_blocks, a.part_sum, a.part_zero, a.ticket, a.out,
                a.cov_bits ? -1.0 : 0.0, a.n_reads, sh_s, sh_z, a.status_out, a.status_a, a.status_b);
  } else if (threadIdx.x == 0) {
    a.part_sum[a.main_blocks + ovf_block] = lsum;
    a.part_zero[a.main_blocks + ovf_block] = zeros;
  }
}

#ifndef GAML_GEN_WAVES
#define GAML_GEN_WAVES 4
#endif
template <bool TICKET, bool GEN = false, bool TL = false>
__global__ __launch_bounds__(kBlock, GEN ? GAML_GEN_WAVES : 5) void paired_score_kernel(PairedArgs a) {
  __shared__ double sh_s[kBlock / 64];
  __shared__ int sh_z[kBlock / 64];
  __shared__ int4 cand[kBlock / 64][2][kOvfCap];
  const int lb = a.total_blocks - 1 - (int)blockIdx.x;
#if GAML_LEAN_ENTRY && defined(__HIP_DEVICE_COMPILE__)
  if (!TL && lb < a.blocks0a && a.memo && !a.cov_bits && a.n_codes == 1) {
    double lsum = 0.0;
    int zeros = 0;
    if (!GAML_TIMING_X(16))
    paired_static4_body<GEN, false, true>(a, SlotRange{0, a.n0a, lb, a.blocks0a}, lsum, zeros);
    block_reduce(lsum, zeros, sh_s, sh_z);
    if (TICKET) grid_finish(lsum, zeros, lb, a.total_blocks, a.part_sum, a.part_zero, a.ticket, a.out, 0.0, a.n_reads, sh_s, sh_z, a.status_out, a.status_a, a.status_b);
    else if (threadIdx.x == 0) { a.part_sum[lb] = lsum; a.part_zero[lb] = zeros; }
    return;
  }
  if (lb < a.main_blocks) paired_main_body<TICKET, GEN, TL>(a, lb, sh_s, sh_z, &cand[0][0][0]);
  else if (GAML_GEN_OFF(16)) { if (threadIdx.x == 0) { a.part_sum[lb] = 0.0; a.part_zero[lb] = 0; } }
  else {
    GAML_FRESH_ARGS(c, a)
    paired_overflow_body<TICKET>(c, lb - c.main_blocks, c.total_blocks - c.main_blocks, sh_s, sh_z, cand);
  }
#else
  if (lb < a.main_blocks) paired_main_body<TICKET, GEN, TL>(a, lb, sh_s, sh_z, &cand[0][0][0]);
  else paired_overflow_body<TICKET>(a, lb - a.main_blocks, a.total_blocks - a.main_blocks, sh_s, sh_z, cand);
#endif
}

constexpr int kMaxSets = 8;
struct SetDev {
  const Occ12* occ12[2];
  const int* multi_off[2];
  const int4* multi[2];
  const double* tfloor_c;
  double tfloor0;
  double two_T, log_two_T;
  double* part_sum;
  int* part_zero;
};
struct MultiSets { int n; int pad_; const unsigned char* chg[2]; SetDev set[kMaxSets]; };

constexpr int kTfCodes = 16;
__device__ __forceinline__ PairedArgs with_set(const PairedArgs& a, const SetDev& sd, const double* tfloor_lds = nullptr) {
  PairedArgs b = a;
#pragma unroll
  for (int mt = 0; mt < 2; mt++) { b.m[mt].occ12 = sd.occ12[mt]; b.occ12[mt] = sd.occ12[mt]; b.m[mt].multi_off = sd.multi_off[mt]; b.m[mt].multi = sd.multi[mt]; }
  b.tfloor_c = tfloor_lds ? tfloor_lds : sd.tfloor_c; b.tfloor0 = sd.tfloor0; b.two_T = sd.two_T; b.log_two_T = sd.log_two_T;
  b.part_sum = sd.part_sum; b.part_zero = sd.part_zero;
  return b;
}

struct MultiKernArgs { PairedArgs a; MultiSets ms; };
#if defined(__HIP_DEVICE_COMPILE__)
#define GAML_CALLEE_ARGS(name, set)                                                                                                  \
  const unsigned long long name##_u = ((unsigned long long)(unsigned)__builtin_amdgcn_readfirstlane((int)(kernargs >> 32)) << 32) |  \
                                      (unsigned)__builtin_amdgcn_readfirstlane((int)kernargs);          \
  const __attribute__((address_space(4))) MultiKernArgs* name##_p = (const __attribute__((address_space(4))) MultiKernArgs*)name##_u; \
  const PairedArgs name##_0 = name##_p->a;                                                                                           \
  const PairedArgs name = (set) >= 0 ? with_set(name##_0, name##_p->ms.set[set]) : name##_0;
#else
#define GAML_CALLEE_ARGS(name, set) const PairedArgs& name = *(const PairedArgs*)nullptr;
#endif
__device__ __noinline__ GenOut compact_general_call(unsigned long long kernargs, int i, int set) {
  GAML_CALLEE_ARGS(a, set)
  GenOut o{0.0, 0};
  compact_general(a, i, o.add, o.zeros);
  return o;
}
__device__ __noinline__ GenOut general_pair_call(unsigned long long kernargs, int i, int dj, int set, int4* lds) {
  GAML_CALLEE_ARGS(a, set)
  GenOut o{0.0, 0};
  int4 priv[2 * kGenCands];
  int4* const cand = lds ? lds : priv;
  const int4 none = make_int4(-1, 0, 0, 0);
  int4 r1[4], r2[4];
  double acc;
  if (dj < 0) {
    const bool four = i >= a.n01;
    const size_t at = four ? (size_t)2 * (a.n01 - a.n0) + (size_t)4 * (i - a.n01) : (size_t)2 * (i - a.n0);
#pragma unroll
    for (int k = 0; k < 4; k++) { const bool has = four || k < 2; r1[k] = has ? a.inl[0][at + (has ? k : 0)] : none; r2[k] = has ? a.inl[1][at + (has ? k : 0)] : none; }
    const uint32_t l12 = a.len12[i - a.n0];
    const int L1 = l12 & 0xffff, L2 = l12 >> 16;
    if (!general_pair_staged<4>(a, r1, r2, L1, L2, acc, cand)) acc = paired_general(a, a.m[0].first[i - a.n0], a.m[1].first[i - a.n0], L1, L2);
    finish_read(a, i, acc, L1, L2, o.add, o.zeros);
  } else {
#pragma unroll
    for (int k = 0; k < 4; k++) { r1[k] = a.dirty_recs[0][4 * (size_t)dj + k]; r2[k] = a.dirty_recs[1][4 * (size_t)dj + k]; }
    const uint32_t l12 = (uint32_t)r1[0].w;
    const int L1 = l12 & 0xffff, L2 = l12 >> 16;
    const int c0 = r2[0].w & 0xff, c1 = (r2[0].w >> 8) & 0xff;
    if (!general_pair_staged<4>(a, r1, r2, L1, L2, acc, cand))
      acc = paired_general_src_masks(a, ListSrc{a.dirty_recs[0] + 4 * (size_t)dj, c0}, ListSrc{a.dirty_recs[1] + 4 * (size_t)dj, c1}, L1, L2);
    finish_read(a, i, acc, L1, L2, o.add, o.zeros);
  }
  return o;
}

template <bool GEN, bool ONE>
__device__ __forceinline__ void paired_compact4_multi_body(const PairedArgs& a, const MultiSets& ms, const SlotRange rg, double* acc_s, int* acc_z, const double* tf) {
  const unsigned stride = (unsigned)rg.blocks * kBlock, n0 = (unsigned)rg.hi;
  const char* const rec0 = (const char*)a.rec8[0];
  const char* const rec1 = (const char*)a.rec8[1];
  const char* const memo = (const char*)a.memo;
  char* const probs = (char*)a.probs;
  const uint32_t l12_one = ONE ? a.len_combo[0] : 0u;
  const double logfloor_one = ONE ? a.logfloor_c[0] : 0.0;
  for (unsigned base = (unsigned)rg.lo + (unsigned)rg.lb * kBlock + threadIdx.x; base < n0; base += 4 * stride) {
// ... 571 lines not shown
```

gaml_amd/csrc/occ_device.hip.h:

```cpp
#pragma once

namespace {

constexpr int kOccMaxDesc = 32;

struct OccDesc { long long off; int slot, start; };
struct OccScatterArgs {
  const OccPre* pool[2];
  Occ12* dst[2];
  int* dst_list[2];
  Occ12* clr[2];
  const int* clr_list[2];
  unsigned* stamp[2];
  int* dup;
  int n_desc, total[2], n_clr[2];
  unsigned serial;
  OccDesc desc[2][kOccMaxDesc];
};

__global__ void __launch_bounds__(kBlock) occ_scatter_kernel(const OccScatterArgs a) {
  const int t0 = a.total[0], t01 = t0 + a.total[1], c0 = t01 + a.n_clr[0], n = c0 + a.n_clr[1];
  for (int i = blockIdx.x * blockDim.x + threadIdx.x; i < n; i += gridDim.x * blockDim.x) {
    if (i < t01) {
      const int mt = i < t0 ? 0 : 1;
// ... 79 lines not shown
      need[mt] = whole[mt];
    }
    D.pool_gen++;
    D.compactions++;
  }
  *bytes = (need[0] + need[1]) * sizeof(OccPre);
  if (need[0] + need[1] == 0) return 0;
  HIP_TRY(c, D.stage.reserve(*bytes));
  OccPre* sp = (OccPre*)D.stage.p;
  for (int mt = 0; mt < 2; mt++) {
    const size_t at = D.pool_used[mt];
    size_t k = 0;
    for (int32_t id : ids) {
      PathMemo& pm = s.planner.memo(id);
      if (!missing(pm, mt)) continue;
      pm.dev_off[mt] = (int64_t)(at + k);
      pm.dev_gen[mt] = D.pool_gen;
      if (!pm.pre[mt].empty()) memcpy(sp + k, pm.pre[mt].data(), pm.pre[mt].size() * sizeof(OccPre));
      k += pm.pre[mt].size();
    }
    if (k) HIP_TRY(c, hipMemcpyAsync(D.pool[mt].as<OccPre>() + at, sp, k * sizeof(OccPre), hipMemcpyHostToDevice, st));
    D.pool_used[mt] = at + k;
    sp += k;
  }
  return 0;
}

int occdev_launch(gaml_hip_ctx* c, PairedSet& s, hipStream_t st, size_t* bytes) {
  PairedSet::OccDev& D = s.occdev;
  const std::vector<int32_t>& ids = s.planner.ids();
  if (D.pool_cap[0] == 0 || D.pool_cap[1] == 0) {
    for (int mt = 0; mt < 2; mt++) {
      size_t all = 0;
      for (int32_t id : ids) all += s.planner.memo(id).pre[mt].size();
      D.pool_cap[mt] = std::max<size_t>(16 * all, (size_t)1 << 10);
      HIP_TRY(c, D.pool[mt].reserve(D.pool_cap[mt] * sizeof(OccPre)));
      D.pool_used[mt] = 0;
    }
    D.pool_gen++;
  }
  size_t n_occ[2] = {0, 0};
  for (int32_t id : ids) for (int mt = 0; mt < 2; mt++) n_occ[mt] += s.planner.memo(id).pre[mt].size();
  const size_t n_windows = std::max(s.mate[0].wins.size(), s.mate[1].wins.size());
  if (int e = occdev_reserve(c, s, n_windows, std::max(n_occ[0], n_occ[1]), st)) return e;
  if (int e = occdev_upload(c, s, st, bytes)) return e;
  HIP_TRY(c, D.dup.reserve(sizeof(int)));
  *(volatile int*)D.dup.p = 0;
  if (++D.serial == 0) {
    for (int mt = 0; mt < 2; mt++) HIP_TRY(c, hipMemsetAsync(D.stamp[mt].p, 0, D.cap_w * sizeof(uint32_t), st));
    D.serial = 1;
  }
  const int cur = (int)(D.serial & 1), other = cur ^ 1;
  OccScatterArgs a;
  memset(&a, 0, sizeof(a));
  a.n_desc = (int)ids.size();
  for (int mt = 0; mt < 2; mt++) {
    a.pool[mt] = D.pool[mt].as<OccPre>();
    a.dst[mt] = D.tab[mt][cur].as<Occ12>();
    a.dst_list[mt] = D.list[mt][cur].as<int>();
    a.clr[mt] = D.tab[mt][other].as<Occ12>();
    a.clr_list[mt] = D.list[mt][other].as<int>();
    a.stamp[mt] = D.stamp[mt].as<unsigned>();
    int start = 0;
    for (size_t k = 0; k < ids.size(); k++) {
      const PathMemo& pm = s.planner.memo(ids[k]);
      a.desc[mt][k] = OccDesc{(long long)pm.dev_off[mt], (int)k, start};
      start += (int)pm.pre[mt].size();
    }
    a.total[mt] = start;
    a.n_clr[mt] = D.list_n[mt][other];
    D.list_n[mt][cur] = start;
    D.list_n[mt][other] = 0;
  }
  a.dup = (int*)D.dup.dev;
  a.serial = D.serial;
  const int items = a.total[0] + a.total[1] + a.n_clr[0] + a.n_clr[1];
  if (items > 0) {
    hipLaunchKernelGGL(occ_scatter_kernel, dim3((unsigned)std::min(512, (items + kBlock - 1) / kBlock)), dim3(kBlock), 0, st, a);
    HIP_TRY(c, hipGetLastError());
  }
  return 0;
}

const Occ12* occdev_table(const PairedSet& s, int mt) { return s.occdev.tab[mt][s.occdev.serial & 1].as<Occ12>(); }

void paired_images_refresh(PairedSet& s) {
  if (!s.occdev.image_stale) return;
  s.planner.rebuild_images(s.mate, s.image);
  s.occdev.image_stale = false;
}

}
```

gaml_amd/csrc/paired_launch.hip.h:

```cpp
#pragma once

namespace {

int paired_host_tabs(gaml_hip_ctx* c, PairedSet& s) {
  if (!s.ins_tab.empty() || !s.floor_tab.empty()) return 0;
  const double c0 = s.cfg.min_prob_start, k0 = s.cfg.min_prob_per_base;
  auto ins = [&](int d) {
    double z = ((double)d - s.cfg.insert_mean) / s.cfg.insert_std;
    return std::exp(-z * z / 2.0) / (std::sqrt(2 * M_PI) * s.cfg.insert_std);
  };
  const int kInsCap = 1 << 22;
  s.ins_tab.clear();
  for (int d = 0; d < kInsCap; d++) {
    double v = ins(d);
    if (v == 0.0 && (double)d > s.cfg.insert_mean) break;
    s.ins_tab.push_back(v);
  }
  if ((int)s.ins_tab.size() >= kInsCap)
    return fail(c, GAML_HIP_EINVAL, "insert_std too large: the insert-size table would exceed 4M entries");
  int smax = s.mate[0].max_len + s.mate[1].max_len;
  s.floor_tab.resize(smax + 1);
  s.logfloor_tab.resize(smax + 1);
  for (int v = 0; v <= smax; v++) {
    s.floor_tab[v] = std::exp(c0 + k0 * v);
    s.logfloor_tab[v] = std::log(s.floor_tab[v]);
    if (!(s.floor_tab[v] > 0.0)) s.floor_positive = false;
  }
  s.covthr_tab.resize(s.mate[1].max_len + 1);
  for (int v = 0; v <= s.mate[1].max_len; v++) s.covthr_tab[v] = std::exp(c0 + k0 * (v + v));
  return 0;
}

int prepare_paired_tables(gaml_hip_ctx* c, PairedSet& s) {
  if (s.tabs_uploaded) return 0;
  if (int e = paired_host_tabs(c, s)) return e;
  size_t total = s.ins_tab.size() + s.floor_tab.size() + s.logfloor_tab.size() + s.covthr_tab.size();
  HIP_TRY(c, s.tabs.reserve(std::max<size_t>(1, total) * sizeof(double)));
  double* d = s.tabs.as<double>();
  size_t at = 0;
  auto up = [&](const std::vector<double>& v) -> hipError_t {
    hipError_t e = v.empty() ? hipSuccess : hipMemcpy(d + at, v.data(), v.size() * sizeof(double), hipMemcpyHostToDevice);
    at += v.size();
    return e;
  };
  HIP_TRY(c, up(s.ins_tab));
  HIP_TRY(c, up(s.floor_tab));
  HIP_TRY(c, up(s.logfloor_tab));
  HIP_TRY(c, up(s.covthr_tab));
  const int64_t n = s.mate[0].n_local();
  HIP_TRY(c, s.probs.reserve(std::max<size_t>(1, n) * sizeof(double)));
  HIP_TRY(c, s.red.init());
  HIP_TRY(c, s.bad.reserve(sizeof(unsigned long long)));
  s.tabs_uploaded = true;
  return 0;
}

int prepare_paired_structure(gaml_hip_ctx* c, PairedSet& s, const int32_t* flat, const int64_t* offs, int32_t n_paths) {
  const bool incremental = !(s.cfg.penalty_constant > 0) && KNOB(c, 12) == 0;
  std::string err;
  if (!s.planner.begin(c->g, s.mate, flat, offs, n_paths, incremental, &err)) return fail(c, GAML_HIP_EINVAL, err);
  return 0;
}

int prepare_paired_tables_host(gaml_hip_ctx* c, PairedSet& s, PairedPrep& p, hipStream_t st = nullptr, bool device_route = false) {
  static const bool trace = getenv("GAML_HIP_TRACE_HOST") != nullptr;
  const double q0 = now_us();
  s.planner.finish(s.mate);
  PairedSet::OccDev& D = s.occdev;
  D.taken = device_route && occdev_route_ok(c, s);
  size_t up_bytes = 0;
  if (D.taken) { if (int e = occdev_launch(c, s, st, &up_bytes)) return e; }
  c->prof[6] = (double)up_bytes;
  const double q1 = now_us();
  const bool cov = s.cfg.penalty_constant > 0;
  p.path_base.assign(1, 0);
  p.start_off.assign(1, 0);
  p.starts.clear();
  if (cov) {
    const PlanView& v = s.planner.view();
    p.path_base.reserve(v.paths.size() + 1);
    p.start_off.reserve(v.paths.size() + 1);
    for (const PathMemo* pm : v.paths) {
      p.starts.insert(p.starts.end(), pm->starts.begin(), pm->starts.end());
      p.start_off.push_back((int32_t)p.starts.size());
      int32_t bits = ((pm->length + 64 + 31) / 32) * 32;
      p.path_base.push_back(p.path_base.back() + bits);
    }
  }
  p.total_bits = p.path_base.back();
  p.n_paths = s.planner.n_paths();
  const double q2 = now_us();
  s.planner.apply(s.mate, s.image, !D.taken, D.image_stale);
  D.image_stale = D.taken;
  if (D.taken) D.dev_calls++; else D.host_calls++;
  p.assembled_records = s.planner.assembled(0) + s.planner.assembled(1);
  p.general = !D.taken && (!s.image[0].general_wids.empty() || !s.image[1].general_wids.empty());
  if (trace) fprintf(stderr, "pass2: finish %.1f us, starts %.1f us, images %.1f us\n", q1 - q0, q2 - q1, now_us() - q2);
  return 0;
}

}
#include "paired_tables.hip.h"
namespace {

double tfloor_for(double floor, double two_T) {
  if (!(floor > 0.0)) return 0.0;
  double x = floor * two_T;
  for (int k = 0; k < 64 && x > 0.0 && (std::nextafter(x, 0.0) / two_T) >= floor; k++) x = std::nextafter(x, 0.0);
  for (int k = 0; k < 64 && (x / two_T) < floor; k++) x = std::nextafter(x, std::numeric_limits<double>::infinity());
  return x;
}

struct PairedLayout { size_t tfloor_off; OccLayout l0, l1; size_t pb_off, so_off, st_off, total; };

PairedLayout paired_layout(const PairedSet& s, const PairedPrep& p, const size_t* pad_to = nullptr) {
  PairedLayout L;
  L.tfloor_off = 0;
  const size_t hdr = align16(256 * sizeof(double));
  L.l0 = layout_image(s.image[0], hdr, pad_to ? pad_to[0] : 0);
  L.l1 = layout_image(s.image[1], L.l0.end, pad_to ? pad_to[1] : 0);
  L.pb_off = L.l1.end; L.so_off = L.st_off = 0; L.total = L.l1.end;
  if (s.cfg.penalty_constant > 0) {
    L.so_off = align16(L.pb_off + p.path_base.size() * sizeof(int32_t));
    L.st_off = align16(L.so_off + p.start_off.size() * sizeof(int32_t));
    L.total = align16(L.st_off + p.starts.size() * sizeof(int32_t));
  }
  return L;
}

void paired_pack_thresholds(const PairedSet& s, const PairedLayout& L, double two_T, char* dst) {
  double tf[256];
  const size_t nc = std::min<size_t>(256, s.pt.len_combo.size());
  for (size_t ci = 0; ci < nc; ci++) {
    const int L0 = (int)(s.pt.len_combo[ci] & 0xffff), L1 = (int)(s.pt.len_combo[ci] >> 16);
    tf[ci] = tfloor_for(s.floor_tab[L0 + L1], two_T);
  }
  if (nc) memcpy(dst + L.tfloor_off, tf, nc * sizeof(double));
}

void paired_pack(const PairedSet& s, const PairedPrep& p, const PairedLayout& L, char* dst) {
  pack_image(s.image[0], L.l0, dst);
  pack_image(s.image[1], L.l1, dst);
  if (s.cfg.penalty_constant > 0) {
    memcpy(dst + L.pb_off, p.path_base.data(), p.path_base.size() * sizeof(int32_t));
    memcpy(dst + L.so_off, p.start_off.data(), p.start_off.size() * sizeof(int32_t));
    memcpy(dst + L.st_off, p.starts.data(), p.starts.size() * sizeof(int32_t));
  }
}

int arena_acquire(gaml_hip_ctx* c, Arena& A, size_t bytes, hipStream_t st, int* slot_out, char** write_ptr) {
  const int k = A.next;
  A.next = (A.next + 1) % kRing;
  if (A.armed[k]) { HIP_TRY(c, hipEventSynchronize(A.done[k])); A.armed[k] = false; }
  if (!A.done[k]) HIP_TRY(c, hipEventCreateWithFlags(&A.done[k], hipEventDisableTiming));
  const bool direct = c->direct_write && KNOB(c, 8) == 0;
  if (bytes > A.cap[k] || A.direct[k] != direct) {
    HIP_TRY(c, hipStreamSynchronize(st));
    if (A.dev[k]) { HIP_TRY(c, hipFree(A.dev[k])); A.dev[k] = nullptr; A.cap[k] = 0; }
    const size_t want = std::max<size_t>(bytes + bytes / 2, (size_t)1 << 20);
    if (direct) HIP_TRY(c, hipExtMallocWithFlags(&A.dev[k], want, hipDeviceMallocFinegrained));
    else HIP_TRY(c, hipMalloc(&A.dev[k], want));
    A.cap[k] = want; A.direct[k] = direct;
  }
  if (direct) *write_ptr = (char*)A.dev[k];
  else { HIP_TRY(c, A.host[k].reserve(bytes)); *write_ptr = (char*)A.host[k].p; }
  *slot_out = k;
  return 0;
}

int arena_commit(gaml_hip_ctx* c, Arena& A, int k, size_t bytes, hipStream_t st) {
  if (A.direct[k]) { _mm_sfence(); return 0; }
  if (bytes == 0) return 0;
  if (KNOB(c, 8) == 1 || (bytes & 15)) { HIP_TRY(c, hipMemcpyAsync(A.dev[k], A.host[k].p, bytes, hipMemcpyHostToDevice, st)); return 0; }
  const int n16 = (int)(bytes / 16);
  hipLaunchKernelGGL(stage_copy_kernel, dim3((unsigned)std::min(64, (n16 + kBlock - 1) / kBlock)), dim3(kBlock), 0, st,
                     (const int4*)A.host[k].dev, (int4*)A.dev[k], n16);
  HIP_TRY(c, hipGetLastError());
// ... 145 lines not shown
  gp.main_blocks = gp.blocks0 + gp.blocks1 + gp.blocks2 + gp.blocks_d;
  gp.ovf_blocks = ovf_total > 0 ? (int)std::min<int64_t>((ovf_total + 3) / 4, kOvfMaxBlocks) : 0;
  gp.total_blocks = gp.main_blocks + gp.ovf_blocks;
  a.blocks0a = gp.blocks0a;
  a.blocks0 = gp.blocks0;
  a.blocks01 = gp.blocks0 + gp.blocks1;
  a.blocks012 = gp.blocks0 + gp.blocks1 + gp.blocks2;
  a.main_blocks = gp.main_blocks;
  a.total_blocks = gp.total_blocks;
}

void paired_set_view(const PairedSet& s, const PairedLayout& L, const char* arena, int32_t total_len, SetDev& sd) {
  const OccLayout* l[2] = {&L.l0, &L.l1};
  for (int mt = 0; mt < 2; mt++) {
    sd.occ12[mt] = (const Occ12*)(arena + l[mt]->direct);
    sd.multi_off[mt] = (const int*)(arena + l[mt]->multi_off);
    sd.multi[mt] = (const int4*)(arena + l[mt]->multi);
  }
  sd.tfloor_c = (const double*)(arena + L.tfloor_off);
  const int tl = total_len == 0 ? 1 : total_len;
  sd.two_T = (double)(2 * tl);
  sd.tfloor0 = paired_tfloor0(s, sd.two_T);
  sd.log_two_T = std::log(sd.two_T);
  sd.part_sum = nullptr; sd.part_zero = nullptr;
}

void paired_apply_set(PairedArgs& a, const SetDev& sd) {
  for (int mt = 0; mt < 2; mt++) { a.m[mt].occ12 = sd.occ12[mt]; a.m[mt].occ = nullptr; a.occ12[mt] = sd.occ12[mt]; a.m[mt].multi_off = sd.multi_off[mt]; a.m[mt].multi = sd.multi[mt]; }
  a.tfloor_c = sd.tfloor_c; a.tfloor0 = sd.tfloor0; a.two_T = sd.two_T; a.log_two_T = sd.log_two_T;
  a.part_sum = sd.part_sum; a.part_zero = sd.part_zero;
}

CovArgs paired_cov_args(const PairedSet& s, const PairedPrep& p, const PairedLayout& L, const char* arena) {
  CovArgs ca;
  ca.bits = s.cov_bits.as<uint32_t>();
  ca.path_base = (const int*)(arena + L.pb_off);
  ca.start_off = (const int*)(arena + L.so_off);
  ca.starts = (const int*)(arena + L.st_off);
  ca.n_paths = p.n_paths;
  ca.total_words = p.total_bits / 32;
  ca.cov_move = s.cfg.step;
  ca.far = s.cfg.insert_mean + 5 * s.cfg.insert_std;
  ca.bad = s.bad.as<unsigned long long>();
  return ca;
}

int paired_host_partials(gaml_hip_ctx* c, PairedSet& s, int first_set, int n_sets, int n_partials, double** d_sum, int** d_zero) {
  const size_t per = (size_t)(4 * kMaxBlocks + kOvfMaxBlocks);
  HIP_TRY(c, s.h_part_sum.reserve(per * sizeof(double) * kMaxSets));
  HIP_TRY(c, s.h_part_zero.reserve(per * sizeof(int) * kMaxSets));
  *d_sum = (double*)s.h_part_sum.dev;
  *d_zero = (int*)s.h_part_zero.dev;
  double* hs = (double*)s.h_part_sum.p;
  int* hz = (int*)s.h_part_zero.p;
  for (int k = first_set; k < first_set + n_sets; k++) {
    for (int b2 = 0; b2 < n_partials; b2++) { hs[(size_t)k * per + b2] = std::numeric_limits<double>::quiet_NaN(); hz[(size_t)k * per + b2] = INT_MIN; }
    s.last_blocks[k] = n_partials;
  }
  s.host_part_stride = per;
  return 0;
}

int launch_paired(gaml_hip_ctx* c, PairedSet& s, PairedPrep& p, int32_t total_len, hipStream_t st, double* out4) {
  const double tpp = now_us();
  if (int e = prepare_paired_tables(c, s)) return e;
  const double tp0 = now_us();
  if (int e = prepare_paired_tables_host(c, s, p, st, true)) return e;
  const double t_after_host = now_us();
  c->prof[1] = t_after_host - tp0;
  gpu_probe(st, c->warm_buf.p, "before table sync");
  if (int e = paired_sync_tables(c, s, st)) return e;
  const double tp1 = now_us();
  c->prof[4] = tp1 - t_after_host;
  if (tp1 - t_after_host > 1000.0 && getenv("GAML_HIP_TRACE_HOST")) fprintf(stderr, "table sync took %.0f us (evaluation %lld of the set, rebuild active %d slice %d)\n", tp1 - t_after_host, (long long)s.eval_count, (int)s.rebuild.active, s.rebuild.next_slice);

  const bool cov = s.cfg.penalty_constant > 0;
  const int tl = total_len == 0 ? 1 : total_len;
  const bool resident = paired_resident_route(c, s);
  PairedLayout L;
  memset(&L, 0, sizeof(L));
  int slot = -1;
  const char* arena = nullptr;
  SetDev sd;
  s.occdev.check_dup = s.occdev.taken;
  if (s.occdev.taken) {
    PairedLayout Lt;
    Lt.tfloor_off = s.persist.off_tfloor;
    paired_pack_thresholds(s, Lt, (double)(2 * tl), (char*)s.persist.dev);
    _mm_sfence();
    paired_persist_view(s, total_len, sd);
    for (int mt = 0; mt < 2; mt++) sd.occ12[mt] = occdev_table(s, mt);
    c->prof[6] += 256.0 * sizeof(double);
  } else if (resident) {
    c->prof[6] = (double)((s.image[0].changed_all || s.image[1].changed_all || !s.persist.valid) ? (s.image[0].occ12.size() + s.image[1].occ12.size()) * sizeof(Occ12)
                                                                                            : (s.image[0].changed.size() + s.image[1].changed.size()) * sizeof(Occ12));
    if (int e = paired_persist_update(c, s, (double)(2 * tl), st)) return e;
    paired_persist_view(s, total_len, sd);
  } else {
    L = paired_layout(s, p);
    char* wp = nullptr;
    if (int e = arena_acquire(c, s.arena, L.total, st, &slot, &wp)) return e;
    paired_pack(s, p, L, wp);
    paired_pack_thresholds(s, L, (double)(2 * tl), wp);
    if (int e = arena_commit(c, s.arena, slot, L.total, st)) return e;
    arena = (const char*)s.arena.dev[slot];
    paired_set_view(s, L, arena, total_len, sd);
    c->prof[6] = (double)L.total;
  }
  const double tp2 = now_us();
  c->prof[3] = tp2 - tp1;

  PairedArgs a;
  GridPlan gp;
  paired_base_args(c, s, a, gp);
  const int64_t n = s.mate[0].n_local();
  if (cov) {
    size_t words = (size_t)p.total_bits / 32;
    if (words * 4 > s.cov_bits.cap) { HIP_TRY(c, hipStreamSynchronize(st)); HIP_TRY(c, s.cov_bits.reserve(std::max<size_t>(4, words * 4))); }
    HIP_TRY(c, hipMemsetAsync(s.cov_bits.p, 0, std::max<size_t>(4, words * 4), st));
    HIP_TRY(c, hipMemsetAsync(s.bad.p, 0, sizeof(unsigned long long), st));
    a.cov_bits = s.cov_bits.as<uint32_t>();
    a.path_base = (const int*)(arena + L.pb_off);
  }
  const bool gen_set = a.n_main > 0 && p.general;
  const int n_partials = gp.total_blocks;
  sd.part_sum = s.red.part_sum.as<double>();
  sd.part_zero = s.red.part_zero.as<int>();
  if (c->host_results && n > 0) { if (int e = paired_host_partials(c, s, 0, 1, n_partials, &sd.part_sum, &sd.part_zero)) return e; }
  s.last_blocks[0] = n > 0 ? n_partials : 0;
  s.last_host_partials = c->host_results;
  s.last_sets = 1;
  paired_apply_set(a, sd);
  a.out = out4;
  a.timeline = nullptr;
  const bool timeline = KNOB(c, 3) == 8;
  if (timeline) {
    HIP_TRY(c, s.h_timeline.reserve((size_t)(4 * kMaxBlocks + kOvfMaxBlocks + 256) * (kBlock / 64) * 8 * sizeof(unsigned long long)));
    memset(s.h_timeline.p, 0, s.h_timeline.cap);
    a.timeline = (unsigned long long*)s.h_timeline.dev;
    s.timeline_waves = a.total_blocks * (kBlock / 64);
  }

  std::pair<hipEvent_t, hipEvent_t>* ev = nullptr;
  if (n > 0) {
    if (c->event_timing && (c->event_tick++ % c->event_every) == 0) { if (int e = take_events(c, &ev)) return e; }
    int fin_mode = c->host_results ? 2 : (KNOB(c, 2) ? KNOB(c, 2) - 1 : 1);
    double* status_out = nullptr;
    if (fin_mode != 2 && c->status_dst && !c->status_done) { status_out = c->status_dst; c->status_done = true; }
    if (fin_mode == 0) { a.status_out = status_out; a.status_a = c->status_a; a.status_b = c->status_b; }
    s.last_total_blocks = n_partials;
    const dim3 grid(a.total_blocks), block(kBlock);
    hipEvent_t e0 = ev ? ev->first : nullptr, e1 = ev ? ev->second : nullptr;
#define GAML_LAUNCH_SCORE(...) hipExtLaunchKernelGGL((paired_score_kernel<__VA_ARGS__>), grid, block, KNOB(c, 1), st, e0, e1, 0, a)
#ifdef GAML_HIP_DEV
    if (timeline) GAML_LAUNCH_SCORE(false, false, true);
    else
#endif
    if (gen_set) { if (fin_mode) GAML_LAUNCH_SCORE(false, true); else GAML_LAUNCH_SCORE(true, true); }
    else if (fin_mode) GAML_LAUNCH_SCORE(false, false);
    else GAML_LAUNCH_SCORE(true, false);
#undef GAML_LAUNCH_SCORE
    HIP_TRY(c, hipGetLastError());
    if (fin_mode == 1) {
      hipLaunchKernelGGL(finish_partials_kernel, dim3(1), dim3(kBlock), 0, st, a.part_sum, a.part_zero, n_partials, out4, cov ? -1.0 : 0.0, (double)n, status_out, c->status_a, c->status_b);
      HIP_TRY(c, hipGetLastError());
    }
  } else {
    s.last_total_blocks = 0;
    if (!c->host_results) HIP_TRY(c, hipMemsetAsync(out4, 0, 4 * sizeof(double), st));
  }
  if (cov && c->defer_cov) {
    int idx = 0;
    for (size_t i = 0; i < c->paireds.size(); i++) if (c->paireds[i].get() == &s) idx = (int)i;
    c->pending_cov.push_back(gaml_hip_ctx::PendingCov{idx, paired_cov_args(s, p, L, arena), out4});
  } else if (cov && n > 0 && p.total_bits > 0) {
    const CovArgs ca = paired_cov_args(s, p, L, arena);
    hipLaunchKernelGGL(coverage_sweep_kernel, dim3(grid_for(ca.total_words)), dim3(kBlock), 0, st, ca);
    HIP_TRY(c, hipGetLastError());
  }
  if (cov && n > 0 && !c->defer_cov) {
    hipLaunchKernelGGL(store_bad_bases_kernel, dim3(1), dim3(64), 0, st, s.bad.as<unsigned long long>(), out4, 1.0);
    HIP_TRY(c, hipGetLastError());
  }
  if (slot >= 0) { if (int e = arena_release(c, s.arena, slot, st)) return e; }
  c->prof[5] = now_us() - tp2;
  if (now_us() - tpp > 5000.0 && getenv("GAML_HIP_TRACE_HOST"))
    fprintf(stderr, "launch_paired: fixed tables %.2f ms, pass 2 %.2f, table sync %.2f, per-call tables %.2f, launches %.2f\n", (tp0 - tpp) * 1e-3, (t_after_host - tp0) * 1e-3,
            (tp1 - t_after_host) * 1e-3, (tp2 - tp1) * 1e-3, (now_us() - tp2) * 1e-3);
  if (!c->event_timing || ev) {
    c->stat_algo_bytes += 16.0 * (double)p.assembled_records + 16.0 * (double)n;
    c->stat_launches++;
  }
  c->t_host_us += t_after_host;
  return 0;
}

bool paired_multi_capable(const gaml_hip_ctx* c, const PairedSet& s) {
  return !(s.cfg.penalty_constant > 0) && KNOB(c, 3) == 0 && KNOB(c, 4) == 0 && s.floor_positive;
}

int launch_paired_multi(gaml_hip_ctx* c, PairedSet& s, int first, int n_sets, const PairedLayout* L, const PairedPrep* preps, const int32_t* total_lens,
                        const char* arena, size_t stride, hipStream_t st, const unsigned char* const* chg = nullptr) {
  PairedArgs a;
  GridPlan gp;
  paired_base_args(c, s, a, gp);
  if (!a.memo) return fail(c, GAML_HIP_ESTATE, "multi-set launch without a memo (caller must check paired_multi_capable)");
  const int64_t n = s.mate[0].n_local();
  bool any_set = false;
  for (int k = first; k < first + n_sets; k++) any_set = any_set || (a.n_main > 0 && preps[k].general);
  const int n_partials = gp.total_blocks;
  double* d_sum = nullptr;
  int* d_zero = nullptr;
  s.last_total_blocks = n > 0 ? n_partials : 0;
  s.last_host_partials = true;
  s.last_sets = first + n_sets;
  if (n == 0) { for (int k = first; k < first + n_sets; k++) s.last_blocks[k] = 0; return 0; }
  if (int e = paired_host_partials(c, s, first, n_sets, n_partials, &d_sum, &d_zero)) return e;
  MultiSets ms;
  memset(&ms, 0, sizeof(ms));
  ms.n = n_sets;
  if (KNOB(c, 11) >= 32) ms.pad_ = (KNOB(c, 11) - 32) & 31;
  if (chg && KNOB(c, 11) < 64) { ms.chg[0] = chg[0]; ms.chg[1] = chg[1]; }
  for (int k = 0; k < n_sets; k++) {
    const int g = first + k;
    paired_set_view(s, L[g], arena + (size_t)g * stride, total_lens[g], ms.set[k]);
    ms.set[k].part_sum = d_sum + (size_t)g * s.host_part_stride;
    ms.set[k].part_zero = d_zero + (size_t)g * s.host_part_stride;
  }
  paired_apply_set(a, ms.set[0]);
  std::pair<hipEvent_t, hipEvent_t>* ev = nullptr;
  if (c->event_timing && (c->event_tick++ % c->event_every) == 0) { if (int e = take_events(c, &ev)) return e; }
  hipEvent_t e0 = ev ? ev->first : nullptr, e1 = ev ? ev->second : nullptr;
  const dim3 grid(a.total_blocks), block(kBlock);
  if (any_set) hipExtLaunchKernelGGL((paired_score_multi_kernel<true>), grid, block, 0, st, e0, e1, 0, a, ms);
  else hipExtLaunchKernelGGL((paired_score_multi_kernel<false>), grid, block, 0, st, e0, e1, 0, a, ms);
  HIP_TRY(c, hipGetLastError());
  if (!c->event_timing || ev) {
    double rec = 0;
    for (int k = first; k < first + n_sets; k++) rec += (double)preps[k].assembled_records;
    c->stat_algo_bytes += 16.0 * rec + 16.0 * (double)n * n_sets;
    c->stat_launches++;
// ... 6 lines not shown
```

include/gaml_hip_debug.h:

```cpp
#ifndef GAML_HIP_DEBUG_H_
#define GAML_HIP_DEBUG_H_

#include "gaml_hip.h"

#ifdef __cplusplus
extern "C" {
#endif

int gaml_hip_debug_sam_logprob(gaml_hip_ctx* ctx, const char* target, int32_t target_len, const char* read, int32_t read_len,
                               const char* sam_line, int64_t sam_len, double mismatch_prob, double* logprob_out,
                               int32_t* band_lo, int32_t* band_hi, int32_t band_cap);
int gaml_hip_debug_sam_shape(const char* sam_line, int64_t len, int32_t total_len, int32_t* out6, uint32_t* ops, int32_t cap);
int32_t gaml_hip_debug_sam_band(const char* sam_line, int64_t len, int32_t total_len, int32_t* fields10, int32_t* row0,
                                int32_t* lo, int32_t* hi, int32_t cap);

int gaml_hip_debug_prepare(gaml_hip_ctx* ctx, const int32_t* paths, const int64_t* path_offs, int32_t n_paths);
int64_t gaml_hip_debug_occurrences(gaml_hip_ctx* ctx, int readset, int mate, int32_t* out5, int64_t cap);
int64_t gaml_hip_debug_table_occurrences(gaml_hip_ctx* ctx, int readset, int mate, int32_t* out5, int64_t cap, int64_t* info3);
int32_t gaml_hip_debug_window_walk(gaml_hip_ctx* ctx, int readset, int mate, int32_t window_id, int32_t* out, int32_t cap);
int gaml_hip_debug_timeline(gaml_hip_ctx* ctx, int rs, unsigned long long* out, int64_t cap_waves);

int gaml_hip_debug_set_knob(gaml_hip_ctx* ctx, int knob, int value);
int gaml_hip_debug_fold_check(gaml_hip_ctx* ctx, int readset, int64_t* out6);
int gaml_hip_debug_radix_sort(gaml_hip_ctx* ctx, uint64_t* keys, uint64_t* vals, int64_t n, int begin_bit, int end_bit, uint64_t* run_max);
int gaml_hip_debug_static_check(gaml_hip_ctx* ctx, int readset, int64_t* out8);
int gaml_hip_debug_tables_check(gaml_hip_ctx* ctx, int readset, int64_t* out8);
int32_t gaml_hip_debug_block_partials(gaml_hip_ctx* ctx, int readset, int32_t set, double* sums, int32_t* zeros, int32_t cap, int32_t* layout8);

int gaml_hip_debug_occ_route(gaml_hip_ctx* ctx, int readset, int64_t* out6);
int gaml_hip_debug_occ_check(gaml_hip_ctx* ctx, int readset, int64_t* out4);

#ifdef __cplusplus
}
#endif
#endif
```

Measured before the change: 62.78 billion reads/s.

## Add direct per-path occurrence tables to skip device table assembly

Adds a direct occurrence path. When one or two disjoint paths are planned, each path's occurrence entries are uploaded once into a per-path dense pool indexed by window id, and the scoring kernels look entries up from both tables through a new DIR template parameter. This skips the occdev_launch merge/build step and its duplicate checking whenever the paths are memoized in the pool. The cost is two loads plus selects per lookup instead of one, and the fast path is forced to the non-ticket, non-generic kernel variant.

```diff
diff --git a/gaml_amd/api.py b/gaml_amd/api.py
--- a/gaml_amd/api.py
+++ b/gaml_amd/api.py
@@ -691,10 +691,11 @@
                 "different_windows": int(out[4]), "orientation": int(out[5]), "distance": int(out[6]), "edits_or_code": int(out[7])}
 
     def debug_occ_route(self, rs):
-        out = np.zeros(6, np.int64)
+        out = np.zeros(8, np.int64)
         self._check(_lib.gaml_hip_debug_occ_route(self._h, rs, out))
         return {"device": int(out[0]), "host": int(out[1]), "fallbacks": int(out[2]), "compactions": int(out[3]),
-                "pool_entries": int(out[4]), "shared_combinations": int(out[5])}
+                "pool_entries": int(out[4]), "shared_combinations": int(out[5]), "direct": int(out[6]),
+                "direct_compactions": int(out[7])}
 
     def debug_occ_check(self, rs):
         out = np.zeros(4, np.int64)
diff --git a/gaml_amd/csrc/ctx.hip.h b/gaml_amd/csrc/ctx.hip.h
--- a/gaml_amd/csrc/ctx.hip.h
+++ b/gaml_amd/csrc/ctx.hip.h
@@ -286,12 +286,19 @@
     size_t shared_next = 0;
     std::vector<uint64_t> key;
     int64_t dev_calls = 0, host_calls = 0, fallbacks = 0, compactions = 0;
+    DevBuf dpool[2];
+    size_t dpool_cap[2] = {0, 0}, dpool_used[2] = {0, 0};
+    uint32_t dpool_gen = 1;
+    PinBuf dstage;
+    bool direct = false;
+    OccDirect dir[2];
+    int64_t direct_calls = 0, dcompactions = 0;
     void release() {
       for (int mt = 0; mt < 2; mt++) {
-        pool[mt].release(); stamp[mt].release();
+        pool[mt].release(); stamp[mt].release(); dpool[mt].release();
         for (int k = 0; k < 2; k++) { tab[mt][k].release(); list[mt][k].release(); }
       }
-      stage.release(); dup.release();
+      stage.release(); dup.release(); dstage.release();
     }
   } occdev;
   int64_t batches_patched = 0, batches_full = 0;
diff --git a/gaml_amd/csrc/debug_api.hip.h b/gaml_amd/csrc/debug_api.hip.h
--- a/gaml_amd/csrc/debug_api.hip.h
+++ b/gaml_amd/csrc/debug_api.hip.h
@@ -308,6 +308,7 @@
   const PairedSet::OccDev& D = c->paireds[c->handles[rs].idx]->occdev;
   out6[0] = D.dev_calls; out6[1] = D.host_calls; out6[2] = D.fallbacks; out6[3] = D.compactions;
   out6[4] = (int64_t)(D.pool_used[0] + D.pool_used[1]); out6[5] = (int64_t)D.shared.size();
+  out6[6] = D.direct_calls; out6[7] = D.dcompactions;
   return GAML_HIP_OK;
 }
 
@@ -326,7 +327,22 @@
     im.build(ps.mate[mt].wins.size(), v, mt);
     const size_t n = im.occ12.size();
     std::vector<Occ12> dev(n);
-    if (n) HIP_TRY(c, hipMemcpy(dev.data(), occdev_table(ps, mt), n * sizeof(Occ12), hipMemcpyDeviceToHost));
+    if (D.direct) {
+      const OccDirect& d = D.dir[mt];
+      std::vector<Occ12> t[2];
+      for (int k = 0; k < 2; k++) {
+        t[k].resize(d.len[k]);
+        HIP_TRY(c, hipMemcpy(t[k].data(), d.base[k], d.len[k] * sizeof(Occ12), hipMemcpyDeviceToHost));
+      }
+      for (size_t w = 0; w < n; w++) {
+        Occ12 r{~0u, ~0u, -1};
+        for (int k = 1; k >= 0; k--) {
+          const unsigned i = (unsigned)w - (unsigned)d.wmin[k];
+          if (i < d.len[k] && t[k][i].hi != ~0u) r = Occ12{t[k][i].lo, t[k][i].hi | ((unsigned)k << 16), t[k][i].rank};
+        }
+        dev[w] = r;
+      }
+    } else if (n) HIP_TRY(c, hipMemcpy(dev.data(), occdev_table(ps, mt), n * sizeof(Occ12), hipMemcpyDeviceToHost));
     for (size_t w = 0; w < n; w++) {
       const Occ12& h = im.occ12[w];
       const Occ12& d = dev[w];
diff --git a/gaml_amd/csrc/host_model.cc b/gaml_amd/csrc/host_model.cc
--- a/gaml_amd/csrc/host_model.cc
+++ b/gaml_amd/csrc/host_model.cc
@@ -882,6 +882,7 @@
       occ_prepack(pm.occ[mt], pm.pre[mt]);
       pm.pre_plain[mt] = occ_pre_plain(pm.pre[mt]);
       pm.dev_off[mt] = -1;
+      pm.dn_off[mt] = -1;
       pm.occ_valid[mt] = true;
     }
   };
diff --git a/gaml_amd/csrc/host_model.h b/gaml_amd/csrc/host_model.h
--- a/gaml_amd/csrc/host_model.h
+++ b/gaml_amd/csrc/host_model.h
@@ -222,6 +222,10 @@
   bool pre_plain[2] = {false, false};
   int64_t dev_off[2] = {-1, -1};
   uint32_t dev_gen[2] = {0, 0};
+  int64_t dn_off[2] = {-1, -1};
+  uint32_t dn_gen[2] = {0, 0};
+  int32_t dwmin[2] = {0, 0}, dlen[2] = {0, 0}, wbits_lo[2] = {0, 0};
+  std::vector<uint64_t> wbits[2];
   int64_t assembled[2] = {0, 0};
   std::vector<int32_t> starts;
   int32_t length = 0;
diff --git a/gaml_amd/csrc/kernels.hip.h b/gaml_amd/csrc/kernels.hip.h
--- a/gaml_amd/csrc/kernels.hip.h
+++ b/gaml_amd/csrc/kernels.hip.h
@@ -9,6 +9,25 @@
 enum { kDsDirty = 0, kDsSpill = 1, kDsTop0 = 2, kDsTop1 = 3, kDsOverflow = 4, kDsSeq = 5, kDsInts = 8 };
 
 __device__ __forceinline__ unsigned long long occ8_of(const Occ12* t, unsigned w) { const Occ12* e = t + w; return (unsigned long long)e->lo | ((unsigned long long)e->hi << 32); }
+
+struct OccDirect { const Occ12* base[2]; int wmin[2]; unsigned len[2]; };
+__device__ __forceinline__ Occ12 occ_direct(const OccDirect& d, unsigned w) {
+  const unsigned i0 = w - (unsigned)d.wmin[0], i1 = w - (unsigned)d.wmin[1];
+  const bool in0 = i0 < d.len[0], in1 = i1 < d.len[1];
+  const Occ12 e0 = d.base[0][in0 ? i0 : 0u];
+  const Occ12 e1 = d.base[1][in1 ? i1 : 0u];
+  const bool p0 = in0 & (e0.hi != ~0u), p1 = in1 & (e1.hi != ~0u);
+  Occ12 r;
+  r.lo = p0 ? e0.lo : (p1 ? e1.lo : ~0u);
+  r.hi = p0 ? e0.hi : (p1 ? e1.hi | (1u << 16) : ~0u);
+  r.rank = p0 ? e0.rank : (p1 ? e1.rank : -1);
+  return r;
+}
+template <bool DIR>
+__device__ __forceinline__ Occ12 occ_entry(const Occ12* t, const OccDirect& d, unsigned w) {
+  if constexpr (DIR) return occ_direct(d, w);
+  else return t[w];
+}
 
 struct MateView {
   const int4* first;
@@ -19,6 +38,7 @@
   const int4* multi;
   const double* mism_pow;
   const double* match_pow;
+  OccDirect dir;
 };
 
 struct PairedArgs {
@@ -83,7 +103,7 @@
 }
 __device__ __forceinline__ int4 mate_occ(const MateView& v, int w) {
   if (v.occ) return v.occ[w];
-  const Occ12 e = v.occ12[w];
+  const Occ12 e = v.occ12 ? v.occ12[w] : occ_direct(v.dir, (unsigned)w);
   return occ_from_compact((unsigned long long)e.lo | ((unsigned long long)e.hi << 32), e.rank);
 }
 
@@ -287,13 +307,13 @@
   bool valid[K], live[K];
 };
 
-template <int K>
+template <int K, bool DIR = false>
 __device__ __forceinline__ bool cands_from_records(const MateView& v, const int4 (&r)[K], RegCands<K>& c) {
   int4 o[K];
   bool multi = false;
   Occ12 e[K];
 #pragma unroll
-  for (int k = 0; k < K; k++) e[k] = v.occ12[r[k].x >= 0 ? r[k].x : 0];
+  for (int k = 0; k < K; k++) e[k] = occ_entry<DIR>(v.occ12, v.dir, r[k].x >= 0 ? r[k].x : 0);
 #pragma unroll
   for (int k = 0; k < K; k++) o[k] = occ_from_compact((unsigned long long)e[k].lo | ((unsigned long long)e[k].hi << 32), e[k].rank);
 #pragma unroll
@@ -542,7 +562,13 @@
   return lb < a.blocks0a ? SlotRange{0, a.n0a, lb, a.blocks0a} : SlotRange{a.n0a, a.n0, lb - a.blocks0a, a.blocks0 - a.blocks0a};
 }
 
-template <bool GEN>
+template <bool DIR>
+__device__ __forceinline__ unsigned long long occ8_at(const PairedArgs& a, int mt, unsigned w) {
+  if constexpr (DIR) { const Occ12 e = occ_direct(a.m[mt].dir, w); return (unsigned long long)e.lo | ((unsigned long long)e.hi << 32); }
+  else return occ8_of(a.occ12[mt], w);
+}
+
+template <bool GEN, bool DIR = false>
 __device__ __forceinline__ void paired_compact_body(const PairedArgs& a, const SlotRange rg, double& lsum, int& zeros) {
   const int stride = rg.blocks * kBlock, hi = rg.hi;
   int i0 = rg.lo + rg.lb * kBlock + threadIdx.x;
@@ -563,10 +589,10 @@
     const bool d0 = c0.r1 == kDirty8, d1 = c1.r1 == kDirty8;
     if (d0) { c0.r1 = kNone8; c0.r2 = kNone8; }
     if (d1) { c1.r1 = kNone8; c1.r2 = kNone8; }
-    c0.o1 = c0.r1 != kNone8 ? occ8_of(a.occ12[0], (unsigned)(c0.r1 & 0xffffff)) : kNone8;
-    c0.o2 = c0.r2 != kNone8 ? occ8_of(a.occ12[1], (unsigned)(c0.r2 & 0xffffff)) : kNone8;
-    c1.o1 = c1.r1 != kNone8 ? occ8_of(a.occ12[0], (unsigned)(c1.r1 & 0xffffff)) : kNone8;
-    c1.o2 = c1.r2 != kNone8 ? occ8_of(a.occ12[1], (unsigned)(c1.r2 & 0xffffff)) : kNone8;
+    c0.o1 = c0.r1 != kNone8 ? occ8_at<DIR>(a, 0, (unsigned)(c0.r1 & 0xffffff)) : kNone8;
+    c0.o2 = c0.r2 != kNone8 ? occ8_at<DIR>(a, 1, (unsigned)(c0.r2 & 0xffffff)) : kNone8;
+    c1.o1 = c1.r1 != kNone8 ? occ8_at<DIR>(a, 0, (unsigned)(c1.r1 & 0xffffff)) : kNone8;
+    c1.o2 = c1.r2 != kNone8 ? occ8_at<DIR>(a, 1, (unsigned)(c1.r2 & 0xffffff)) : kNone8;
     CompactPrep q0, q1;
     compact_prep(a, c0, q0);
     compact_prep(a, c1, q1);
@@ -606,7 +632,7 @@
   return state;
 }
 
-template <bool GEN, bool TL = false, bool ONE = false>
+template <bool GEN, bool TL = false, bool ONE = false, bool DIR = false>
 __device__ __forceinline__ void paired_compact4_body(const PairedArgs& a, const SlotRange rg, double& lsum, int& zeros) {
   const unsigned stride = (unsigned)rg.blocks * kBlock, n0 = (unsigned)rg.hi;
   unsigned long long* tl = TL ? a.timeline + ((size_t)blockIdx.x * (kBlock / 64) + (threadIdx.x >> 6)) * 8 : nullptr;
@@ -630,9 +656,14 @@
     GAML_STAMP(2, r1[0].x ^ r1[1].x ^ r1[2].x ^ r1[3].x ^ r2[0].x ^ r2[3].x)
 #pragma unroll
     for (int k = 0; k < 4; k++) {
+      if constexpr (DIR) {
+        const Occ12 e1 = occ_direct(a.m[0].dir, r1[k].y != ~0u ? (r1[k].x & 0xffffffu) : 0u), e2 = occ_direct(a.m[1].dir, r2[k].y != ~0u ? (r2[k].x & 0xffffffu) : 0u);
+        o1[k] = make_uint2(e1.lo, e1.hi); o2[k] = make_uint2(e2.lo, e2.hi);
+      } else {
       const Occ12* e1 = (const Occ12*)(occ0 + (r1[k].y != ~0u ? (r1[k].x & 0xffffffu) : 0u) * 12u);
       const Occ12* e2 = (const Occ12*)(occ1 + (r2[k].y != ~0u ? (r2[k].x & 0xffffffu) : 0u) * 12u);
       o1[k] = make_uint2(e1->lo, e1->hi); o2[k] = make_uint2(e2->lo, e2->hi);
+      }
     }
     GAML_STAMP(3, o1[0].x ^ o1[1].x ^ o1[2].x ^ o1[3].x ^ o2[0].x ^ o2[3].x)
     int state[4];
@@ -670,8 +701,8 @@
         const int i = (int)(base + k * stride);
         Compact1 d;
         compact_load(a, i, true, d);
-        d.o1 = d.r1 != kNone8 ? occ8_of(a.occ12[0], (unsigned)(d.r1 & 0xffffff)) : kNone8;
-        d.o2 = d.r2 != kNone8 ? occ8_of(a.occ12[1], (unsigned)(d.r2 & 0xffffff)) : kNone8;
+        d.o1 = d.r1 != kNone8 ? occ8_at<DIR>(a, 0, (unsigned)(d.r1 & 0xffffff)) : kNone8;
+        d.o2 = d.r2 != kNone8 ? occ8_at<DIR>(a, 1, (unsigned)(d.r2 & 0xffffff)) : kNone8;
         const uint32_t l = a.len_combo[d.lc];
         d.L1 = l & 0xffff; d.L2 = l >> 16;
         CompactPrep q;
@@ -718,7 +749,7 @@
   }
 }
 
-template <bool GEN, bool TL = false, bool ONE = false>
+template <bool GEN, bool TL = false, bool ONE = false, bool DIR = false>
 __device__ __forceinline__ void paired_static4_body(const PairedArgs& a, const SlotRange rg, double& lsum, int& zeros) {
   constexpr int P = GAML_STATIC_P;
   const unsigned stride = (unsigned)rg.blocks * kBlock, n0 = (unsigned)rg.hi;
@@ -749,9 +780,14 @@
 #pragma unroll
     for (int k = 0; k < P; k++) {
       const unsigned w1 = (r1[k].x & 0xffffffu) & (0u - (unsigned)(r1[k].y != ~0u)), w2 = (r2[k].x & 0xffffffu) & (0u - (unsigned)(r2[k].y != ~0u));
+      if constexpr (DIR) {
+        const Occ12 e1 = occ_direct(a.m[0].dir, w1), e2 = occ_direct(a.m[1].dir, w2);
+        o1[k] = make_uint2(e1.lo, e1.hi); o2[k] = make_uint2(e2.lo, e2.hi);
+      } else {
       const Occ12* e1 = (const Occ12*)(occ0 + w1 * 12u);
       const Occ12* e2 = (const Occ12*)(occ1 + w2 * 12u);
       o1[k] = make_uint2(e1->lo, e1->hi); o2[k] = make_uint2(e2->lo, e2->hi);
+      }
       if (GAML_TIMING_X(1)) { o1[k] = make_uint2(r1[k].x >> 8, 0u); o2[k] = make_uint2(r1[k].x >> 8, 0u); }
     }
     const unsigned nbase = base + P * stride;
@@ -971,7 +1007,7 @@
     finish_read(a, i, acc, L1, L2, lsum, zeros, cap);
 }
 
-template <int K, bool GEN>
+template <int K, bool GEN, bool DIR = false>
 __device__ __forceinline__ void paired_regs_body(const PairedArgs& a, int lb, int slot_lo, int slot_hi, int block_lo, int block_hi,
                                                  double& lsum, int& zeros, unsigned long long* tl = nullptr, int4* wave_lds = nullptr) {
   bool first_pair = true;
@@ -987,7 +1023,7 @@
     for (int k = 0; k < K; k++) { r1[k] = a.inl[0][at + k]; r2[k] = a.inl[1][at + k]; }
     if (tl && first_pair) { asm volatile("s_waitcnt vmcnt(0)" ::: "memory"); if ((threadIdx.x & 63) == 0) tl[2] = (unsigned long long)wall_clock64() + (r1[0].x == 0x12345 ? 1 : 0); }
     RegCands<K> x, y;
-    const bool m1 = cands_from_records<K>(a.m[0], r1, x), m2 = cands_from_records<K>(a.m[1], r2, y);
+    const bool m1 = cands_from_records<K, DIR>(a.m[0], r1, x), m2 = cands_from_records<K, DIR>(a.m[1], r2, y);
     if (tl && first_pair) { asm volatile("s_waitcnt vmcnt(0)" ::: "memory"); if ((threadIdx.x & 63) == 0) tl[3] = (unsigned long long)wall_clock64() + (x.pos[0] == 0x12345 ? 1 : 0); }
     const bool dirty = r1[0].x == kDirtyWid;
     const bool general = !dirty && (m1 || m2);
@@ -1013,7 +1049,7 @@
   }
 }
 
-template <bool GEN>
+template <bool GEN, bool DIR = false>
 __device__ __forceinline__ void paired_delta_body(const PairedArgs& a, int db, int delta_blocks, double& lsum, int& zeros, int4* wave_lds = nullptr) {
   for (int dj = db * kBlock + threadIdx.x; dj < a.dstate[kDsDirty]; dj += delta_blocks * kBlock) {
     const int i = a.dirty_slots[dj];
@@ -1028,7 +1064,7 @@
       if (sp < 0) {
         RegCands<2> x, y;
         const int4 q0[2] = {r0[0], r0[1]}, q1[2] = {r1[0], r1[1]};
-        const bool m0 = cands_from_records<2>(a.m[0], q0, x), m1 = cands_from_records<2>(a.m[1], q1, y);
+        const bool m0 = cands_from_records<2, DIR>(a.m[0], q0, x), m1 = cands_from_records<2, DIR>(a.m[1], q1, y);
         general = m0 || m1;
         if (!general) score_cands_and_finish<2>(a, i, l12, x, y, lsum, zeros);
       }
@@ -1036,7 +1072,7 @@
 #pragma unroll
       for (int k = 2; k < 4; k++) { r0[k] = a.dirty_recs[0][4 * (size_t)dj + k]; r1[k] = a.dirty_recs[1][4 * (size_t)dj + k]; }
       RegCands<4> x, y;
-      const bool m0 = cands_from_records<4>(a.m[0], r0, x), m1 = cands_from_records<4>(a.m[1], r1, y);
+      const bool m0 = cands_from_records<4, DIR>(a.m[0], r0, x), m1 = cands_from_records<4, DIR>(a.m[1], r1, y);
       general = m0 || m1;
       if (!general) score_cands_and_finish<4>(a, i, l12, x, y, lsum, zeros);
     }
@@ -1077,7 +1113,7 @@
   }
 }
 
-template <bool TICKET, bool GEN, bool TL>
+template <bool TICKET, bool GEN, bool TL, bool DIR = false>
 __device__ __forceinline__ void paired_main_body(const PairedArgs& a, int lb, double* sh_s, int* sh_z, int4* gen_lds) {
   double lsum = 0.0;
   int zeros = 0;
@@ -1091,8 +1127,8 @@
     const SlotRange rg = compact_range(c, lb);
     const bool stat = wide && lb < c.blocks0a;
     if (!TL && wide && c.n_codes == 1) {
-      if (stat) paired_static4_body<GEN, false, true>(c, rg, lsum, zeros);
-      else paired_compact4_body<GEN, false, true>(c, rg, lsum, zeros);
+      if (stat) paired_static4_body<GEN, false, true, DIR>(c, rg, lsum, zeros);
+      else paired_compact4_body<GEN, false, true, DIR>(c, rg, lsum, zeros);
     } else {
       __shared__ uint32_t sh_combo[256];
       __shared__ double sh_floor[256], sh_logfloor[256], sh_tfloor[256];
@@ -1101,21 +1137,21 @@
       PairedArgs b = c;
       b.len_combo = sh_combo; b.floor_c = sh_floor; b.logfloor_c = sh_logfloor; b.tfloor_c = sh_tfloor;
       if (TL && (threadIdx.x & 63) == 0) tl[1] = wall_clock64();
-      if (stat) paired_static4_body<GEN, TL>(b, rg, lsum, zeros);
-      else if (wide) paired_compact4_body<GEN, TL>(b, rg, lsum, zeros);
-      else paired_compact_body<GEN>(b, rg, lsum, zeros);
+      if (stat) paired_static4_body<GEN, TL, false, DIR>(b, rg, lsum, zeros);
+      else if (wide) paired_compact4_body<GEN, TL, false, DIR>(b, rg, lsum, zeros);
+      else paired_compact_body<GEN, DIR>(b, rg, lsum, zeros);
     }
   } else {
     int4* const wave_lds = GEN ? gen_lds + (threadIdx.x >> 6) * 2 * kOvfCap : nullptr;
     if (lb < a.blocks01) {
       GAML_FRESH_ARGS(c, a)
-      paired_regs_body<2, GEN>(c, lb, c.n0, c.n01, c.blocks0, c.blocks01, lsum, zeros, tl, wave_lds);
+      paired_regs_body<2, GEN, DIR>(c, lb, c.n0, c.n01, c.blocks0, c.blocks01, lsum, zeros, tl, wave_lds);
     } else if (lb < a.blocks012) {
       GAML_FRESH_ARGS(c, a)
-      paired_regs_body<4, GEN>(c, lb, c.n01, c.n_main, c.blocks01, c.blocks012, lsum, zeros, nullptr, wave_lds);
+      paired_regs_body<4, GEN, DIR>(c, lb, c.n01, c.n_main, c.blocks01, c.blocks012, lsum, zeros, nullptr, wave_lds);
     } else {
       GAML_FRESH_ARGS(c, a)
-      paired_delta_body<GEN>(c, lb - c.blocks012, c.main_blocks - c.blocks012, lsum, zeros, wave_lds);
+      paired_delta_body<GEN, DIR>(c, lb - c.blocks012, c.main_blocks - c.blocks012, lsum, zeros, wave_lds);
     }
   }
   block_reduce(lsum, zeros, sh_s, sh_z);
@@ -1146,7 +1182,7 @@
 
 constexpr int kOvfMaxBlocks = 1024;
 
-template <class Src>
+template <bool DIR, class Src>
 __device__ __forceinline__ int wave_gather(const MateView& v, const Src& src, int4* lds, int lane) {
   const int cnt = src.count();
   int total = 0;
@@ -1156,7 +1192,7 @@
     int4 r = make_int4(-1, 0, 0, 0), o = make_int4(0, 0, -1, 0);
     if (k < cnt) {
       r = src.get(k);
-      if (r.x >= 0) { const Occ12 e = v.occ12[r.x]; o = occ_from_compact((unsigned long long)e.lo | ((unsigned long long)e.hi << 32), e.rank); }
+      if (r.x >= 0) { const Occ12 e = occ_entry<DIR>(v.occ12, v.dir, (unsigned)r.x); o = occ_from_compact((unsigned long long)e.lo | ((unsigned long long)e.hi << 32), e.rank); }
       if (o.z >= 0) mine = o.w >= 0 ? 1 : v.multi_off[-o.w] - v.multi_off[-o.w - 1];
     }
     int incl = mine;
@@ -1178,10 +1214,10 @@
   return total;
 }
 
-template <class Src>
+template <bool DIR = false, class Src>
 __device__ __forceinline__ double wave_score_pair(const PairedArgs& a, const Src& s1, const Src& s2, int L1, int L2, int4* c1, int4* c2, int lane) {
-  const int n1 = wave_gather(a.m[0], s1, c1, lane);
-  const int n2 = wave_gather(a.m[1], s2, c2, lane);
+  const int n1 = wave_gather<DIR>(a.m[0], s1, c1, lane);
+  const int n2 = wave_gather<DIR>(a.m[1], s2, c2, lane);
   double acc = 0.0;
   if (n1 < 0 || n2 < 0) {
     if (lane == 0) acc = paired_general_src(a, s1, s2, L1, L2);
@@ -1219,7 +1255,7 @@
   return acc;
 }
 
-template <bool TICKET>
+template <bool TICKET, bool DIR = false>
 __device__ __forceinline__ void paired_overflow_body(const PairedArgs& a, int ovf_block, int ovf_blocks, double* sh_s, int* sh_z,
                                                      int4 (*cand)[2][kOvfCap]) {
   const int lane = threadIdx.x & 63, wave = threadIdx.x >> 6;
@@ -1238,7 +1274,7 @@
       const uint32_t l12 = a.len12[i - a.n0];
       if (r1.x == kDirtyWid) continue;
       const int L1 = l12 & 0xffff, L2 = l12 >> 16;
-      const double acc = wave_score_pair(a, TableSrc{&a.m[0], r1}, TableSrc{&a.m[1], r2}, L1, L2, c1, c2, lane);
+      const double acc = wave_score_pair<DIR>(a, TableSrc{&a.m[0], r1}, TableSrc{&a.m[1], r2}, L1, L2, c1, c2, lane);
       if (lane == 0) finish_read(a, i, acc, L1, L2, lsum, zeros);
     } else {
       const int sp = item - n_table;
@@ -1246,7 +1282,7 @@
       const uint32_t l12 = i < a.n0 ? a.len_combo[a.len_code[i]] : a.len12[i - a.n0];
       const int L1 = l12 & 0xffff, L2 = l12 >> 16;
       const int2 g0 = a.spill_rng[0][sp], g1 = a.spill_rng[1][sp];
-      const double acc = wave_score_pair(a, ListSrc{a.spill_recs[0] + g0.x, g0.y}, ListSrc{a.spill_recs[1] + g1.x, g1.y}, L1, L2, c1, c2, lane);
+      const double acc = wave_score_pair<DIR>(a, ListSrc{a.spill_recs[0] + g0.x, g0.y}, ListSrc{a.spill_recs[1] + g1.x, g1.y}, L1, L2, c1, c2, lane);
       if (lane == 0) finish_read(a, i, acc, L1, L2, lsum, zeros);
     }
   }
@@ -1263,8 +1299,9 @@
 #ifndef GAML_GEN_WAVES
 #define GAML_GEN_WAVES 4
 #endif
-template <bool TICKET, bool GEN = false, bool TL = false>
+template <bool TICKET, bool GEN = false, bool TL = false, bool DIR = false>
 __global__ __launch_bounds__(kBlock, GEN ? GAML_GEN_WAVES : 5) void paired_score_kernel(PairedArgs a) {
+  static_assert(!(GEN && DIR), "the direct route has no window that occurs several times");
   __shared__ double sh_s[kBlock / 64];
   __shared__ int sh_z[kBlock / 64];
   __shared__ int4 cand[kBlock / 64][2][kOvfCap];
@@ -1274,21 +1311,21 @@
     double lsum = 0.0;
     int zeros = 0;
     if (!GAML_TIMING_X(16))
-    paired_static4_body<GEN, false, true>(a, SlotRange{0, a.n0a, lb, a.blocks0a}, lsum, zeros);
+    paired_static4_body<GEN, false, true, DIR>(a, SlotRange{0, a.n0a, lb, a.blocks0a}, lsum, zeros);
     block_reduce(lsum, zeros, sh_s, sh_z);
     if (TICKET) grid_finish(lsum, zeros, lb, a.total_blocks, a.part_sum, a.part_zero, a.ticket, a.out, 0.0, a.n_reads, sh_s, sh_z, a.status_out, a.status_a, a.status_b);
     else if (threadIdx.x == 0) { a.part_sum[lb] = lsum; a.part_zero[lb] = zeros; }
     return;
   }
-  if (lb < a.main_blocks) paired_main_body<TICKET, GEN, TL>(a, lb, sh_s, sh_z, &cand[0][0][0]);
+  if (lb < a.main_blocks) paired_main_body<TICKET, GEN, TL, DIR>(a, lb, sh_s, sh_z, &cand[0][0][0]);
   else if (GAML_GEN_OFF(16)) { if (threadIdx.x == 0) { a.part_sum[lb] = 0.0; a.part_zero[lb] = 0; } }
   else {
     GAML_FRESH_ARGS(c, a)
-    paired_overflow_body<TICKET>(c, lb - c.main_blocks, c.total_blocks - c.main_blocks, sh_s, sh_z, cand);
+    paired_overflow_body<TICKET, DIR>(c, lb - c.main_blocks, c.total_blocks - c.main_blocks, sh_s, sh_z, cand);
   }
 #else
-  if (lb < a.main_blocks) paired_main_body<TICKET, GEN, TL>(a, lb, sh_s, sh_z, &cand[0][0][0]);
-  else paired_overflow_body<TICKET>(a, lb - a.main_blocks, a.total_blocks - a.main_blocks, sh_s, sh_z, cand);
+  if (lb < a.main_blocks) paired_main_body<TICKET, GEN, TL, DIR>(a, lb, sh_s, sh_z, &cand[0][0][0]);
+  else paired_overflow_body<TICKET, DIR>(a, lb - a.main_blocks, a.total_blocks - a.main_blocks, sh_s, sh_z, cand);
 #endif
 }
 
diff --git a/gaml_amd/csrc/occ_device.hip.h b/gaml_amd/csrc/occ_device.hip.h
--- a/gaml_amd/csrc/occ_device.hip.h
+++ b/gaml_amd/csrc/occ_device.hip.h
@@ -185,6 +185,93 @@
   return 0;
 }
 
+constexpr size_t kDirMaxEntries = (size_t)1 << 22;
+
+void occdir_index(PathMemo& pm, int mt) {
+  const std::vector<OccPre>& pre = pm.pre[mt];
+  int32_t lo = INT32_MAX, hi = -1;
+  for (const OccPre& e : pre) { lo = std::min(lo, e.wid); hi = std::max(hi, e.wid); }
+  if (hi < 0) lo = hi = 0;
+  pm.dwmin[mt] = lo;
+  pm.dlen[mt] = hi - lo + 1;
+  pm.wbits_lo[mt] = lo >> 6;
+  pm.wbits[mt].assign((size_t)((hi >> 6) - (lo >> 6) + 1), 0ull);
+  for (const OccPre& e : pre) pm.wbits[mt][(e.wid >> 6) - pm.wbits_lo[mt]] |= 1ull << (e.wid & 63);
+}
+
+bool occdir_disjoint(const PathMemo& a, const PathMemo& b, int mt) {
+  const int32_t lo = std::max(a.wbits_lo[mt], b.wbits_lo[mt]);
+  const int32_t hi = std::min(a.wbits_lo[mt] + (int32_t)a.wbits[mt].size(), b.wbits_lo[mt] + (int32_t)b.wbits[mt].size());
+  for (int32_t w = lo; w < hi; w++)
+    if (a.wbits[mt][w - a.wbits_lo[mt]] & b.wbits[mt][w - b.wbits_lo[mt]]) return false;
+  return true;
+}
+
+int occdir_prepare(gaml_hip_ctx* c, PairedSet& s, hipStream_t st, size_t* bytes, bool* ok) {
+  PairedSet::OccDev& D = s.occdev;
+  const std::vector<int32_t>& ids = s.planner.ids();
+  *ok = false;
+  if (ids.size() > 2 || KNOB(c, 21) != 0 || KNOB(c, 3) == 8) return 0;
+  auto missing = [&](const PathMemo& pm, int mt) { return pm.dn_off[mt] < 0 || pm.dn_gen[mt] != D.dpool_gen; };
+  size_t need[2] = {0, 0}, whole[2] = {0, 0};
+  for (size_t k = 0; k < ids.size(); k++)
+    for (int mt = 0; mt < 2; mt++) {
+      PathMemo& pm = s.planner.memo(ids[k]);
+      if (missing(pm, mt)) { occdir_index(pm, mt); need[mt] += (size_t)pm.dlen[mt]; }
+      whole[mt] += (size_t)pm.dlen[mt];
+    }
+  if (ids.size() == 2) {
+    if (ids[0] == ids[1]) return 0;
+    const PathMemo &a = s.planner.memo(ids[0]), &b = s.planner.memo(ids[1]);
+    if (!occdir_disjoint(a, b, 0) || !occdir_disjoint(a, b, 1)) return 0;
+  }
+  if (2 * whole[0] > kDirMaxEntries || 2 * whole[1] > kDirMaxEntries) return 0;
+  if (D.dpool_used[0] + need[0] > D.dpool_cap[0] || D.dpool_used[1] + need[1] > D.dpool_cap[1]) {
+    HIP_TRY(c, hipStreamSynchronize(st));
+    for (int mt = 0; mt < 2; mt++) {
+      if (2 * whole[mt] > D.dpool_cap[mt]) {
+        D.dpool_cap[mt] = std::min(kDirMaxEntries, std::max<size_t>(16 * whole[mt], 2 * D.dpool_cap[mt]));
+        HIP_TRY(c, D.dpool[mt].reserve(D.dpool_cap[mt] * sizeof(Occ12)));
+      }
+      D.dpool_used[mt] = 0;
+    }
+    if (D.dpool_gen++ > 1) D.dcompactions++;
+    need[0] = need[1] = 0;
+    for (int32_t id : ids) for (int mt = 0; mt < 2; mt++) need[mt] += (size_t)s.planner.memo(id).dlen[mt];
+  }
+  *bytes = (need[0] + need[1]) * sizeof(Occ12);
+  if (need[0] + need[1] > 0) {
+    HIP_TRY(c, D.dstage.reserve(*bytes));
+    Occ12* sp = (Occ12*)D.dstage.p;
+    for (int mt = 0; mt < 2; mt++) {
+      const size_t at = D.dpool_used[mt];
+      size_t k = 0;
+      for (int32_t id : ids) {
+        PathMemo& pm = s.planner.memo(id);
+        if (!missing(pm, mt)) continue;
+        Occ12* t = sp + k;
+        for (int32_t j = 0; j < pm.dlen[mt]; j++) t[j] = Occ12{~0u, ~0u, -1};
+        for (const OccPre& e : pm.pre[mt]) t[e.wid - pm.dwmin[mt]] = Occ12{e.lo, e.hi, e.rank};
+        pm.dn_off[mt] = (int64_t)(at + k);
+        pm.dn_gen[mt] = D.dpool_gen;
+        k += (size_t)pm.dlen[mt];
+      }
+      if (k) HIP_TRY(c, hipMemcpyAsync(D.dpool[mt].as<Occ12>() + at, sp, k * sizeof(Occ12), hipMemcpyHostToDevice, st));
+      D.dpool_used[mt] = at + k;
+      sp += k;
+    }
+  }
+  for (int mt = 0; mt < 2; mt++)
+    for (int k = 0; k < 2; k++) {
+      const PathMemo& pm = s.planner.memo(ids[std::min<size_t>(k, ids.size() - 1)]);
+      D.dir[mt].base[k] = D.dpool[mt].as<Occ12>() + pm.dn_off[mt];
+      D.dir[mt].wmin[k] = pm.dwmin[mt];
+      D.dir[mt].len[k] = (unsigned)pm.dlen[mt];
+    }
+  *ok = true;
+  return 0;
+}
+
 const Occ12* occdev_table(const PairedSet& s, int mt) { return s.occdev.tab[mt][s.occdev.serial & 1].as<Occ12>(); }
 
 void paired_images_refresh(PairedSet& s) {
diff --git a/gaml_amd/csrc/paired_launch.hip.h b/gaml_amd/csrc/paired_launch.hip.h
--- a/gaml_amd/csrc/paired_launch.hip.h
+++ b/gaml_amd/csrc/paired_launch.hip.h
@@ -68,8 +68,10 @@
   s.planner.finish(s.mate);
   PairedSet::OccDev& D = s.occdev;
   D.taken = device_route && occdev_route_ok(c, s);
+  D.direct = false;
   size_t up_bytes = 0;
-  if (D.taken) { if (int e = occdev_launch(c, s, st, &up_bytes)) return e; }
+  if (D.taken) { if (int e = occdir_prepare(c, s, st, &up_bytes, &D.direct)) return e; }
+  if (D.taken && !D.direct) { if (int e = occdev_launch(c, s, st, &up_bytes)) return e; }
   c->prof[6] = (double)up_bytes;
   const double q1 = now_us();
   const bool cov = s.cfg.penalty_constant > 0;
@@ -93,6 +95,7 @@
   s.planner.apply(s.mate, s.image, !D.taken, D.image_stale);
   D.image_stale = D.taken;
   if (D.taken) D.dev_calls++; else D.host_calls++;
+  if (D.direct) D.direct_calls++;
   p.assembled_records = s.planner.assembled(0) + s.planner.assembled(1);
   p.general = !D.taken && (!s.image[0].general_wids.empty() || !s.image[1].general_wids.empty());
   if (trace) fprintf(stderr, "pass2: finish %.1f us, starts %.1f us, images %.1f us\n", q1 - q0, q2 - q1, now_us() - q2);
@@ -404,14 +407,15 @@
   int slot = -1;
   const char* arena = nullptr;
   SetDev sd;
-  s.occdev.check_dup = s.occdev.taken;
+  const bool direct = s.occdev.taken && s.occdev.direct;
+  s.occdev.check_dup = s.occdev.taken && !direct;
   if (s.occdev.taken) {
     PairedLayout Lt;
     Lt.tfloor_off = s.persist.off_tfloor;
     paired_pack_thresholds(s, Lt, (double)(2 * tl), (char*)s.persist.dev);
     _mm_sfence();
     paired_persist_view(s, total_len, sd);
-    for (int mt = 0; mt < 2; mt++) sd.occ12[mt] = occdev_table(s, mt);
+    for (int mt = 0; mt < 2; mt++) sd.occ12[mt] = direct ? nullptr : occdev_table(s, mt);
     c->prof[6] += 256.0 * sizeof(double);
   } else if (resident) {
     c->prof[6] = (double)((s.image[0].changed_all || s.image[1].changed_all || !s.persist.valid) ? (s.image[0].occ12.size() + s.image[1].occ12.size()) * sizeof(Occ12)
@@ -453,6 +457,7 @@
   s.last_host_partials = c->host_results;
   s.last_sets = 1;
   paired_apply_set(a, sd);
+  if (direct) for (int mt = 0; mt < 2; mt++) a.m[mt].dir = s.occdev.dir[mt];
   a.out = out4;
   a.timeline = nullptr;
   const bool timeline = KNOB(c, 3) == 8;
@@ -478,7 +483,8 @@
     if (timeline) GAML_LAUNCH_SCORE(false, false, true);
     else
 #endif
-    if (gen_set) { if (fin_mode) GAML_LAUNCH_SCORE(false, true); else GAML_LAUNCH_SCORE(true, true); }
+    if (direct) GAML_LAUNCH_SCORE(false, false, false, true);
+    else if (gen_set) { if (fin_mode) GAML_LAUNCH_SCORE(false, true); else GAML_LAUNCH_SCORE(true, true); }
     else if (fin_mode) GAML_LAUNCH_SCORE(false, false);
     else GAML_LAUNCH_SCORE(true, false);
 #undef GAML_LAUNCH_SCORE
diff --git a/include/gaml_hip_debug.h b/include/gaml_hip_debug.h
--- a/include/gaml_hip_debug.h
+++ b/include/gaml_hip_debug.h
@@ -27,7 +27,7 @@
 int gaml_hip_debug_tables_check(gaml_hip_ctx* ctx, int readset, int64_t* out8);
 int32_t gaml_hip_debug_block_partials(gaml_hip_ctx* ctx, int readset, int32_t set, double* sums, int32_t* zeros, int32_t cap, int32_t* layout8);
 
-int gaml_hip_debug_occ_route(gaml_hip_ctx* ctx, int readset, int64_t* out6);
+int gaml_hip_debug_occ_route(gaml_hip_ctx* ctx, int readset, int64_t* out8);
 int gaml_hip_debug_occ_check(gaml_hip_ctx* ctx, int readset, int64_t* out4);
 
 #ifdef __cplusplus
```

Result: faster. 70.55 billion reads/s (median of 6 runs) (+12.4%).
